# ingonyama-zk/gnark-icicle

Measured on AMD Instinct MI355X. Metric: BN254 G1 MSM Mpoints/s (2^20 points per GPU, sharded MSM), higher is better.
Workload: dtype u32 limbs (BN254 Fp/Fr Montgomery, integer); 1 GPU; BN254 G1 MSM 2^20 random points/scalars per GPU (BASELINE configs[1]); points_per_gpu=1048576, total_points=1048576, parallelism=msm-shard1

## Files before the change

### gnark-icicle_amd/csrc/msm.hpp

```cpp
#pragma once
#include <algorithm>
#include <cmath>
#include <cstddef>
#include <cstdint>
#include <cstdlib>
#include <hip/hip_runtime.h>
#include "curves.hpp"

struct gm_ctx;
struct gm_msm_pending;

namespace gm {
struct Arena;
constexpr uint32_t S2_BIG = 1u << 16;
constexpr uint32_t S2_STAGE = 6144;
struct SortGeom {
  uint32_t T = 0, F = 0, G = 0, NC = 0, NS = 0;
  size_t M = 0;
  bool compact = false;
};
inline bool sort_compact_fits(uint32_t F, uint32_t G, size_t npts) {
  uint32_t vb = 1;
  while (npts && ((npts - 1) >> (vb - 1))) vb++;
  return F + G + vb <= 32;
}
int msm_sort_digits(gm_ctx* ctx, Arena& arena, const SortGeom& g, size_t n, uint32_t W, uint32_t nb,
                    uint32_t shared_stride, const uint32_t* dig, const uint32_t* scount, uint32_t* keys_out,
                    uint32_t* vals_out, uint32_t* offsets);

constexpr uint32_t PRECOMP_LAYOUT = 2;
struct MsmPrecomp {
  uint32_t c = 0, W = 0;
  uint32_t narrow = 0;
  size_t stride = 0;
};
inline uint32_t precomp_narrow(uint32_t c, uint32_t W, int bits) {
  const long long e = (long long)c * W - (bits + 1);
  if (e <= 0) return 0;
  return (uint32_t)(e < (long long)W - 1 ? e : (long long)W - 1);
}

MsmPrecomp msm_choose_precomp(size_t n, int bits);

inline int choose_window(size_t n, int bits) {
  int best = 8;
  double best_cost = 1e300;
  for (int c = 8; c <= 20; c++) {
    const double W = (double)((bits + 1 + c - 1) / c);
    const double cost = (double)n * W + 3.0 * W * (double)(1u << (c - 1));
    if (cost < best_cost) {
      best_cost = cost;
      best = c;
    }
  }
  return best;
}

constexpr int GLV_HALF_BITS = 127;

struct MsmPlanGeom {
  size_t n = 0;
  int bits = 0;
  uint32_t c = 0, W = 0, nb = 0, Wred = 0, total = 0;
  uint32_t wn = 0;
  size_t npts = 0, M = 0;
  SortGeom sg;
};
inline const char* msm_plan_geom(size_t n0, int fr_bits, bool glv, const MsmPrecomp* pre, int c_override,
                                 MsmPlanGeom& g) {
  g = MsmPlanGeom();
  size_t n = n0;
  g.bits = fr_bits;
  if (glv) {
    n = 2 * n0;
    g.bits = GLV_HALF_BITS;
  }
  g.n = n;
  if (n >= (size_t(1) << 31)) return "msm: n must be < 2^31";
  const bool shared = pre && pre->c;
  if (shared && (pre->stride < n || (size_t)pre->W * pre->stride >= (size_t(1) << 31) || pre->narrow >= pre->W ||
                 (size_t)pre->c * pre->W - pre->narrow < (size_t)fr_bits + 1))
    return "msm: precomputed point set does not cover this MSM";
  const uint32_t c = shared ? pre->c : (c_override ? (uint32_t)c_override : (uint32_t)choose_window(n, g.bits));
  const uint32_t W = shared ? pre->W : (uint32_t)(g.bits + 1 + c - 1) / c;
  g.c = c;
  g.W = W;
  g.nb = 1u << (c - 1);
  g.Wred = shared ? 1 : W;
  g.total = g.Wred * g.nb;
  g.npts = shared ? (size_t)W * pre->stride : n;
  const size_t M = (size_t)W * n;
  g.M = M;
  if (M >= (size_t(1) << 31)) return "msm: n * windows must be < 2^31";
  SortGeom& sg = g.sg;
  sg.T = g.total;
  sg.M = M;
  sg.F = 4;
  const double bin_entries = glv || shared ? 4096.0 : 2048.0;
  while (sg.F < 13 && (double)M * std::ldexp(1.0, (int)sg.F + 1) <= bin_entries * sg.T) sg.F++;
  auto bins = [&](uint32_t sh) { return (uint32_t)(((uint64_t)sg.T + (1ull << sh) - 1) >> sh); };
  auto touched = [&](uint32_t sh) { return shared ? bins(sh) : std::max(1u, g.nb >> sh); };
  const char* ming = getenv("GM_MSM_SORT_MING");
  sg.G = ming ? (uint32_t)std::min(10, std::max(0, atoi(ming))) : 0u;
  const uint32_t max_touched = (shared && M < (size_t(1) << 24)) ? 8192u : 512u;
  while (sg.G < 10 && (touched(sg.F + sg.G) > max_touched || bins(sg.F + sg.G) > 8192)) sg.G++;
  while (sg.G && sg.F + sg.G > 31) sg.G--;
  sg.NC = bins(sg.F);
  sg.NS = bins(sg.F + sg.G);
  if (sg.NS > 8192) return "msm: too many buckets for the sort";
  const char* wide = getenv("GM_MSM_SORT_WIDE");
  sg.compact = !(wide && atoi(wide) > 0) && sort_compact_fits(sg.F, sg.G, g.npts);
  g.wn = shared ? W - pre->narrow : W;
  if (!shared && !glv) {
    const uint32_t narrow = c * W - (uint32_t)(g.bits + 1);
    if (narrow < W) g.wn = W - narrow;
  }
  return nullptr;
}

inline void msm_seg_geom(uint32_t Wred, uint32_t nb, uint32_t& L, uint32_t& nseg) {
  uint32_t Lwant = 4;
  while (Lwant < 32 && (size_t)Wred * nb / (2 * Lwant) >= (size_t(1) << 17)) Lwant *= 2;
  L = nb >= Lwant ? Lwant : nb;
  nseg = nb / L;
}

constexpr uint32_t BS_THREADS = 256;
struct MsmTreeGeom {
  static constexpr uint32_t MAX_LEVELS = 24;
  uint32_t levels = 0, lg[MAX_LEVELS] = {}, Q = 2;
};
inline bool msm_tree_geom(uint32_t nseg, size_t xyzz_bytes, MsmTreeGeom& g) {
  g = MsmTreeGeom();
  const size_t slot_budget = (96u << 10) / xyzz_bytes;
  uint32_t m = nseg, Q = 2;
  while (m > 1) {
    uint32_t lg = 0;
    while ((2u << lg) <= m && (size_t)(2u << lg) * Q <= slot_budget && (1u << lg) * (Q + 1) <= 2 * BS_THREADS) lg++;
    if (lg == 0 || g.levels == MsmTreeGeom::MAX_LEVELS) return false;
    g.lg[g.levels++] = lg;
    Q += lg;
    m >>= lg;
  }
  g.Q = Q;
  return true;
}

constexpr uint32_t MSM_SKIP = 0x7fffffffu;

struct MsmPlan {
  uint32_t c = 0, W = 0, nb = 0, total = 0;
  uint32_t Wred = 0;
  size_t n = 0, M = 0;
  size_t npts = 0;
  int bits = 0;
  uint32_t wn = 0;
  uint32_t* keys = nullptr;
  uint32_t* vals = nullptr;
  uint32_t* offsets = nullptr;
  uint32_t T = 0;
  size_t max_pieces = 0, max_parts = 0;
  uint4* pieces = nullptr;
  uint32_t* pcount = nullptr;
  uint32_t* pbase = nullptr;
  uint32_t* partb = nullptr;
};
constexpr uint32_t PIECE_PART = 0x80000000u;
constexpr uint32_t PIECE_MAX_LEN = 128;
uint32_t msm_piece_len(const gm_ctx* ctx, size_t M);
int msm_piece_plan(gm_ctx* ctx, Arena& arena, MsmPlan& plan, uint32_t T);
template <class C>
int msm_plan(gm_ctx* ctx, Arena& arena, const void* scalars_dev, size_t n, const MsmPrecomp* pre,
             MsmPlan& plan, bool glv = false, bool pieces = true, bool keys = true);
bool msm_glv_on(const gm_ctx* ctx, bool g2, size_t n);
template <class C, bool G2>
int msm_run(gm_ctx* ctx, const MsmPlan& plan, const void* points_internal,
            typename GroupSel<C, G2>::HF (&jac_out)[3]);

struct MsmTail {
  size_t n = 0, M = 0;
  uint32_t c = 0, W = 0, Wr = 0, nb = 0, total = 0, L = 0, nseg = 0, K = 0, Q = 2;
  uint32_t wn = 0;
  const uint32_t* keys = nullptr;
  const uint32_t* offsets = nullptr;
  uint32_t T = 0;
  size_t max_parts = 0;
  const uint32_t *pcount = nullptr, *pbase = nullptr, *partb = nullptr;
  void *buckets = nullptr, *pfirst = nullptr, *plast = nullptr, *nodes_a = nullptr, *nodes_b = nullptr;
  void *wsum = nullptr, *errw = nullptr;
  uint8_t* stage = nullptr;
  gm_ctx* stage_ctx = nullptr;
  int stage_idx = -1;
  hipEvent_t done = nullptr;
  void release_stage();
  MsmTail() = default;
  MsmTail(const MsmTail&) = delete;
  MsmTail& operator=(const MsmTail&) = delete;
  ~MsmTail() {
    if (done) hipEventDestroy(done);
    release_stage();
  }
};
template <class C, bool G2>
int msm_launch(gm_ctx* ctx, Arena& arena, const MsmPlan& plan, const void* points_internal, MsmTail& t);
template <class C, bool G2>
int msm_finish(gm_ctx* ctx, MsmTail& t, typename GroupSel<C, G2>::HF (&jac_out)[3]);
template <class C, bool G2>
int msm_device_launch(gm_ctx* ctx, Arena& arena, const void* scalars_dev, const void* points_dev, size_t n,
                      bool points_internal, const MsmPrecomp* pre, MsmTail& t,
                      hipEvent_t inputs_read = nullptr);

template <class C, bool G2>
int msm_device(gm_ctx* ctx, const void* scalars_dev, const void* points_dev, size_t n,
               typename GroupSel<C, G2>::HF (&jac_out)[3], bool points_internal = false,
               const MsmPrecomp* pre = nullptr);
template <class C, bool G2>
int msm_prepare_points(gm_ctx* ctx, const void* gnark_points, size_t n, void* dst);
template <class C, bool G2>
int msm_precompute_points(gm_ctx* ctx, const void* gnark_points, size_t n, const MsmPrecomp& pre, void* dst);
template <class C, bool G2>
size_t msm_internal_point_bytes();
int msm_async_queue(gm_ctx* ctx, int curve, int g2, const void* scalars_dev, const void* points_dev, size_t n,
                    bool prepared, gm_msm_pending** out);
}
```

### gnark-icicle_amd/csrc/msm_impl.hpp

```cpp
#pragma once
#include "curves.hpp"
#include "msm.hpp"
#include "pair_fp2.hpp"
#include "runtime.hpp"

#include <hip/hip_ext.h>

#include <cmath>
#include <cstdlib>
#include <cstring>
#include <type_traits>

namespace gm {

template <class Fr>
GM_DEV uint32_t window_bits(const FeG<Fr>& k, uint32_t bit, uint32_t mask) {
  const uint32_t idx = bit >> 5, sh = bit & 31;
  uint32_t lo = 0, hi = 0;
#pragma unroll
  for (int i = 0; i < Fr::NG; i++) {
    lo = (idx == (uint32_t)i) ? k.w[i] : lo;
    hi = (idx + 1 == (uint32_t)i) ? k.w[i] : hi;
  }
  const uint64_t v = ((uint64_t)hi << 32) | lo;
  return (uint32_t)(v >> sh) & mask;
}

template <class Fr>
GM_DEV FeG<Fr> load_scalar_canonical(const uint32_t* __restrict__ s, uint32_t i) {
  return fe_pack(fe_gnark_to_canonical(fe_load_g<Fr>(s, i)));
}

struct DigitGeom {
  uint32_t n, c, W, nb, shared_stride, F;
  uint32_t wn;
};
GM_HD void window_geom(uint32_t c, uint32_t wn, uint32_t w, uint32_t& off, uint32_t& cw) {
  off = w * c - (w > wn ? w - wn : 0u);
  cw = w >= wn ? c - 1 : c;
}

constexpr uint32_t DG_THREADS = 1024, DG_PPT = 4;

template <class Fr>
__global__ void __launch_bounds__(1024) k_msm_digits(const uint32_t* __restrict__ scalars, DigitGeom g,
                                                     uint32_t NC, uint32_t* __restrict__ dig,
                                                     uint32_t* __restrict__ ccount) {
  extern __shared__ uint32_t dg_lds[];
  const uint32_t t = threadIdx.x;
  for (uint32_t q = t; q < NC; q += DG_THREADS) dg_lds[q] = 0;
  __syncthreads();
  const uint32_t base = blockIdx.x * DG_THREADS * DG_PPT;
  for (uint32_t r = 0; r < DG_PPT; r++) {
    const uint32_t i = base + r * DG_THREADS + t;
    if (i >= g.n) break;
    const FeG<Fr> k = load_scalar_canonical<Fr>(scalars, i);
    uint32_t carry = 0;
    for (uint32_t w = 0; w < g.W; w++) {
      uint32_t off, cw;
      window_geom(g.c, g.wn, w, off, cw);
      const uint32_t raw = window_bits(k, off, (1u << cw) - 1) + carry;
      uint32_t d, neg;
      if (raw > (1u << (cw - 1))) {
        d = (1u << cw) - raw;
        carry = 1;
        neg = 1;
      } else {
        d = raw;
        carry = 0;
        neg = 0;
      }
      dig[(size_t)w * g.n + i] = d ? (d - 1) | (neg << 31) : 0xffffffffu;
      if (d) atomicAdd(&dg_lds[(g.shared_stride ? d - 1 : w * g.nb + d - 1) >> g.F], 1u);
    }
  }
  __syncthreads();
  for (uint32_t q = t; q < NC; q += DG_THREADS)
    if (dg_lds[q]) atomicAdd(&ccount[q], dg_lds[q]);
}

struct GlvBn254 {
  GM_HD static constexpr uint64_t g1(int i) {
    constexpr uint64_t a[5] = {0x163b4843cb4b9a5eull, 0x149d540fd5e495ccull, 0x5398fd0300ff6565ull,
                               0x4ccef014a773d2d2ull, 0x0000000000000002ull};
    return a[i];
  }
  GM_HD static constexpr uint64_t g2(int i) {
    constexpr uint64_t a[4] = {0x8fa7d32d2fafba64ull, 0x6eb9c714773a6ef2ull, 0xd91d232ec7e0b3d7ull,
                               0x0000000000000002ull};
    return a[i];
  }
  static constexpr uint64_t A1_LO = 0x8211bbeb7d4f1128ull, A1_HI = 0x6f4d8248eeb859fcull;
  static constexpr uint64_t A2 = 0x89d3256894d213e3ull;
  static constexpr uint64_t B2_LO = 0x0be4e1541221250bull, B2_HI = 0x6f4d8248eeb859fdull;
  GM_HD static constexpr uint32_t beta29(int i) {
    constexpr uint32_t a[9] = {0x18ccb791u, 0x175b1c3au, 0x0b83d6e2u, 0x0e8ed071u, 0x1282bee2u,
                               0x04220e84u, 0x1fe4017fu, 0x15084d4au, 0x00169119u};
    return a[i];
  }
  GM_HD static constexpr uint32_t beta29_g2(int i) {
    constexpr uint32_t a[9] = {0x0a337995u, 0x158d1d23u, 0x189c9b98u, 0x12fa4e45u, 0x185faadcu,
                               0x0176f16du, 0x0eed93bau, 0x14291140u, 0x000c0afeu};
    return a[i];
  }
};

struct GlvBls377 {
  GM_HD static constexpr uint64_t g(int i) {
    constexpr uint64_t a[5] = {0x5cc5a03b7b820d29ull, 0x3366fc876f25c6b5ull, 0x7f72ed32af90182cull,
                               0xb3f7aa969fd37160ull, 0x0000000000000003ull};
    return a[i];
  }
  static constexpr uint64_t LAM_LO = 0x0a11800000000000ull, LAM_HI = 0x452217cc90000001ull;
  GM_HD static constexpr uint32_t beta29(int i) {
    constexpr uint32_t a[14] = {0x1c8a7893u, 0x0b7d08f2u, 0x06b88506u, 0x162aa2edu, 0x1c5fdf80u,
                                0x11b95a22u, 0x03b86dd7u, 0x1191f770u, 0x10701220u, 0x1501c11fu,
                                0x1cee88bbu, 0x118d05ecu, 0x06f2fa26u, 0x00000000u};
    return a[i];
  }
  GM_HD static constexpr uint32_t beta29_g2(int i) {
    constexpr uint32_t a[14] = {0x098a903fu, 0x0deef70eu, 0x0bd62e43u, 0x12fc3bfau, 0x0de940feu,
                                0x047b8e82u, 0x17ec1b27u, 0x1a776815u, 0x120a67b5u, 0x0a70d0c4u,
                                0x0271dc9au, 0x182f7308u, 0x19602487u, 0x00000000u};
    return a[i];
  }
};

struct GlvBls381 {
  GM_HD static constexpr uint64_t g(int i) {
    constexpr uint64_t a[5] = {0xda5e4f8d896c72ddull, 0x389f49a7268bf7a3ull, 0x63f6e522f6cfee30ull,
                               0x7c6becf1e01faaddull, 0x0000000000000001ull};
    return a[i];
  }
  static constexpr uint64_t LAM_LO = 0x00000000ffffffffull, LAM_HI = 0xac45a4010001a402ull;
  GM_HD static constexpr uint64_t r(int i) {
    constexpr uint64_t a[4] = GM_BLS12381_FR_P64;
    return a[i];
  }
  GM_HD static constexpr uint64_t half(int i) {
    constexpr uint64_t a[4] = {0x7fffffff80000000ull, 0xa9ded2017fff2dffull, 0x199cec0404d0ec02ull,
                               0x39f6d3a994cebea4ull};
    return a[i];
  }
  static constexpr unsigned __int128 MAX_HALF =
      ((((unsigned __int128)LAM_HI << 64) | LAM_LO) + 1) / 2 + 1;
  static_assert(MAX_HALF < ((unsigned __int128)1 << GLV_HALF_BITS),
                "the halves of the balanced split must fit the digits of a GLV plan");
  GM_HD static constexpr uint32_t beta29(int i) {
    constexpr uint32_t a[14] = {0x1195dfebu, 0x1b04e484u, 0x06026044u, 0x086070a2u, 0x1fd68858u,
                                0x137e9670u, 0x06871e67u, 0x1e736664u, 0x083b24f6u, 0x08a70373u,
                                0x02a012fdu, 0x0112f94bu, 0x18a2733cu, 0x00000003u};
    return a[i];
  }
  GM_HD static constexpr uint32_t beta29_g2(int i) {
    constexpr uint32_t a[14] = {0x0abf79e7u, 0x194b14ebu, 0x1ceb16a6u, 0x1845cd5du, 0x0c814568u,
                                0x199ca109u, 0x13ee6ee1u, 0x05d123e5u, 0x0dfbdce2u, 0x010ecb54u,
                                0x0d9337edu, 0x1daaf4b0u, 0x146806fbu, 0x0000000cu};
    return a[i];
  }
};

template <class P>
struct GlvBeta;
template <>
struct GlvBeta<Bn254Fp> {
  GM_HD static constexpr uint32_t g1(int i) { return GlvBn254::beta29(i); }
  GM_HD static constexpr uint32_t g2(int i) { return GlvBn254::beta29_g2(i); }
};
template <>
struct GlvBeta<Bls377Fp> {
  GM_HD static constexpr uint32_t g1(int i) { return GlvBls377::beta29(i); }
  GM_HD static constexpr uint32_t g2(int i) { return GlvBls377::beta29_g2(i); }
};
template <>
struct GlvBeta<Bls381Fp> {
  GM_HD static constexpr uint32_t g1(int i) { return GlvBls381::beta29(i); }
  GM_HD static constexpr uint32_t g2(int i) { return GlvBls381::beta29_g2(i); }
};

template <class P>
GM_DEV Fe<P> glv_phi_x(const Fe<P>& x) {
  Fe<P> b;
#pragma unroll
  for (int j = 0; j < P::N; j++) b.v[j] = GlvBeta<P>::g1(j);
  return fe_mul(x, b);
}
template <class P, int B>
GM_DEV Fe2<P, B> glv_phi_x(const Fe2<P, B>& x) {
  Fe<P> b;
#pragma unroll
  for (int j = 0; j < P::N; j++) b.v[j] = GlvBeta<P>::g2(j);
  return {fe_mul(x.a0, b), fe_mul(x.a1, b)};
}

template <int NG, class GF>
GM_DEV unsigned __int128 glv_mulshift(const uint64_t (&k)[4], GF g) {
  uint64_t t[4 + NG] = {};
#pragma unroll
  for (int i = 0; i < 4; i++) {
    uint64_t carry = 0;
#pragma unroll
    for (int j = 0; j < NG; j++) {
      const unsigned __int128 v = (unsigned __int128)k[i] * g(j) + t[i + j] + carry;
      t[i + j] = (uint64_t)v;
      carry = (uint64_t)(v >> 64);
    }
    t[i + NG] = carry;
  }
  return ((unsigned __int128)t[7] << 64) | t[6];
}

template <class Fr>
GM_DEV void emit_digits(const FeG<Fr>& k, uint32_t flip, uint32_t i, const DigitGeom& g, uint32_t* __restrict__ dig,
                        uint32_t* lds) {
  const uint32_t mask = (1u << g.c) - 1;
  uint32_t carry = 0;
  for (uint32_t w = 0; w < g.W; w++) {
    const uint32_t raw = window_bits(k, w * g.c, mask) + carry;
    uint32_t d, neg;
    if (raw > g.nb) {
      d = (1u << g.c) - raw;
      carry = 1;
      neg = 1;
    } else {
      d = raw;
      carry = 0;
      neg = 0;
    }
    dig[(size_t)w * g.n + i] = d ? (d - 1) | ((neg ^ flip) << 31) : 0xffffffffu;
    if (d) atomicAdd(&lds[(w * g.nb + d - 1) >> g.F], 1u);
  }
}

template <class C>
struct Glv {
  static constexpr bool ok = false;
  static constexpr bool signed_k1 = false;
};
template <>
struct Glv<CurveBN254> {
  static constexpr bool ok = true;
  static constexpr bool signed_k1 = false;
  using U = unsigned __int128;
  GM_DEV static void split(const uint64_t (&k64)[4], U& k1, U& k2, uint32_t& neg2) {
    const U c1 = glv_mulshift<5>(k64, GlvBn254::g1);
    const U c2 = glv_mulshift<4>(k64, GlvBn254::g2);
    const U a1 = ((U)GlvBn254::A1_HI << 64) | GlvBn254::A1_LO;
    const U b2 = ((U)GlvBn254::B2_HI << 64) | GlvBn254::B2_LO;
    const U klo = ((U)k64[1] << 64) | k64[0];
    k1 = klo - c1 * a1 - c2 * (U)GlvBn254::A2;
    k2 = c1 * (U)GlvBn254::A2 - c2 * b2;
    neg2 = (uint32_t)(k2 >> 127);
    if (neg2) k2 = (U)0 - k2;
  }
};
template <>
struct Glv<CurveBLS12377> {
  static constexpr bool ok = true;
  static constexpr bool signed_k1 = false;
  using U = unsigned __int128;
  GM_DEV static void split(const uint64_t (&k64)[4], U& k1, U& k2, uint32_t& neg2) {
    U q = glv_mulshift<5>(k64, GlvBls377::g);
    const U lam = ((U)GlvBls377::LAM_HI << 64) | GlvBls377::LAM_LO;
    const U klo = ((U)k64[1] << 64) | k64[0];
    U r = klo - q * lam;
    if (r >= lam) {
      r -= lam;
      q += 1;
    }
    k1 = r;
    k2 = q;
    neg2 = 0;
  }
};

template <>
struct Glv<CurveBLS12381> {
  static constexpr bool ok = true;
  static constexpr bool signed_k1 = true;
  using U = unsigned __int128;
  GM_DEV static void split(const uint64_t (&k64)[4], U& k1, uint32_t& neg1, U& k2, uint32_t& neg2) {
    uint64_t kk[4], borrow = 0, b2 = 0;
#pragma unroll
    for (int i = 0; i < 4; i++) {
      const U d = (U)GlvBls381::half(i) - k64[i] - borrow;
      borrow = (uint64_t)(d >> 127) & 1;
      const U e = (U)GlvBls381::r(i) - k64[i] - b2;
      b2 = (uint64_t)(e >> 127) & 1;
      kk[i] = (uint64_t)e;
    }
    const uint32_t flip = (uint32_t)borrow;
#pragma unroll
    for (int i = 0; i < 4; i++) kk[i] = flip ? kk[i] : k64[i];
    U q = glv_mulshift<5>(kk, GlvBls381::g);
    const U lam = ((U)GlvBls381::LAM_HI << 64) | GlvBls381::LAM_LO;
    const U klo = ((U)kk[1] << 64) | kk[0];
    U r0 = klo - q * lam;
    neg1 = 0;
    if (r0 > (lam >> 1)) {
      r0 = lam - r0;
      q += 1;
      neg1 = 1;
    }
    k1 = r0;
    k2 = q;
    neg1 ^= flip;
    neg2 = flip;
  }
};

template <class C>
__global__ void __launch_bounds__(1024) k_msm_digits_glv(const uint32_t* __restrict__ scalars, DigitGeom g,
                                                         uint32_t n0, uint32_t NC, uint32_t* __restrict__ dig,
                                                         uint32_t* __restrict__ ccount) {
  using Fr = typename C::Fr;
  extern __shared__ uint32_t dg_lds[];
  const uint32_t t = threadIdx.x;
  for (uint32_t q = t; q < NC; q += DG_THREADS) dg_lds[q] = 0;
  __syncthreads();
  const uint32_t base = blockIdx.x * DG_THREADS * DG_PPT;
  for (uint32_t r = 0; r < DG_PPT; r++) {
    const uint32_t i = base + r * DG_THREADS + t;
    if (i >= n0) break;
    const FeG<Fr> k = load_scalar_canonical<Fr>(scalars, i);
    uint64_t k64[4];
#pragma unroll
    for (int j = 0; j < 4; j++) k64[j] = (uint64_t)k.w[2 * j] | ((uint64_t)k.w[2 * j + 1] << 32);
    unsigned __int128 k1, k2;
    uint32_t neg1 = 0, neg2;
    if constexpr (Glv<C>::signed_k1) Glv<C>::split(k64, k1, neg1, k2, neg2);
    else Glv<C>::split(k64, k1, k2, neg2);
    FeG<Fr> m1, m2;
#pragma unroll
    for (int j = 0; j < Fr::NG; j++) {
      m1.w[j] = j < 4 ? (uint32_t)(k1 >> (32 * j)) : 0u;
      m2.w[j] = j < 4 ? (uint32_t)(k2 >> (32 * j)) : 0u;
    }
    emit_digits<Fr>(m1, neg1, i, g, dig, dg_lds);
    emit_digits<Fr>(m2, neg2, n0 + i, g, dig, dg_lds);
  }
  __syncthreads();
  for (uint32_t q = t; q < NC; q += DG_THREADS)
    if (dg_lds[q]) atomicAdd(&ccount[q], dg_lds[q]);
}

template <class F, bool GLV>
__global__ void __launch_bounds__(256) k_msm_convert_points_lds(const uint32_t* __restrict__ src, size_t n,
                                                                uint32_t* __restrict__ dst) {
  constexpr int PW = 2 * Coord<F>::WORDS;
  constexpr uint32_t Q = PW / 4;
  static_assert(PW % 4 == 0, "points are whole uint4s");
  __shared__ uint4 tile[256 * (Q + 1)];
  const size_t b0 = (size_t)blockIdx.x * 256;
  const uint32_t np = (uint32_t)min((size_t)256, n - b0);
  const uint32_t t = threadIdx.x;
  const uint4* s = reinterpret_cast<const uint4*>(src) + b0 * Q;
  for (uint32_t q = t; q < np * Q; q += 256) tile[(q / Q) * (Q + 1) + q % Q] = s[q];
  __syncthreads();
  uint32_t* mine = reinterpret_cast<uint32_t*>(tile + t * (Q + 1));
  Affine<F> a;
  if (t < np) {
    a = load_affine_gnark<F>(mine);
    store_affine_packed<F>(mine, a);
  }
  __syncthreads();
  uint4* d = reinterpret_cast<uint4*>(dst) + b0 * Q;
  for (uint32_t q = t; q < np * Q; q += 256) d[q] = tile[(q / Q) * (Q + 1) + q % Q];
  if constexpr (GLV) {
    __syncthreads();
    if (t < np) {
      a.x = glv_phi_x(a.x);
      store_affine_packed<F>(mine, a);
    }
    __syncthreads();
    uint4* d2 = reinterpret_cast<uint4*>(dst) + (n + b0) * Q;
    for (uint32_t q = t; q < np * Q; q += 256) d2[q] = tile[(q / Q) * (Q + 1) + q % Q];
  }
}

template <class F>
__global__ void __launch_bounds__(256) k_msm_convert_points(const uint32_t* __restrict__ src, size_t n,
                                                            uint32_t* __restrict__ dst) {
  const size_t i = (size_t)blockIdx.x * blockDim.x + threadIdx.x;
  if (i >= n) return;
  constexpr int PW = 2 * Coord<F>::WORDS;
  store_affine_packed<F>(dst + i * PW, load_affine_gnark<F>(src + i * PW));
}

template <class F>
__global__ void __launch_bounds__(128) k_msm_precompute(uint32_t* __restrict__ pts, size_t n, size_t stride,
                                                        uint32_t c, uint32_t W, uint32_t wn) {
  const size_t i = (size_t)blockIdx.x * blockDim.x + threadIdx.x;
  if (i >= n) return;
  constexpr int PW = 2 * Coord<F>::WORDS;
  const Affine<F> P = load_affine_packed<F>(pts + i * PW);
  Affine<F> zero;
  zero.x = FOps<F>::zero();
  zero.y = FOps<F>::zero();
  if (aff_is_inf(P)) {
    for (uint32_t w = 1; w < W; w++) store_affine_packed<F>(pts + (w * stride + i) * PW, zero);
    return;
  }
  XYZZ<F> acc;
  acc.x = P.x;
  acc.y = P.y;
  acc.zz = FOps<F>::one();
  acc.zzz = FOps<F>::one();
  for (uint32_t w = 1; w < W; w++) {
    const uint32_t cw = (w - 1 >= wn) ? c - 1 : c;
    for (uint32_t k = 0; k < cw; k++) acc = xyzz_dbl(acc);
    Affine<F> r = zero;
    if (!xyzz_is_inf(acc)) {
      const F t = fe_inv(fe_mul(acc.zz, acc.zzz));
      r.x = fe_mul(acc.x, fe_mul(t, acc.zzz));
      r.y = fe_mul(acc.y, fe_mul(t, acc.zz));
    }
    store_affine_packed<F>(pts + (w * stride + i) * PW, r);
  }
}

template <int PW>
struct PackedPt {
  uint32_t w[PW];
};
template <int PW>
GM_DEV PackedPt<PW> load_packed_pt(const uint32_t* __restrict__ src) {
  static_assert(PW % 4 == 0, "packed points are whole 16-byte chunks");
  PackedPt<PW> r;
#pragma unroll
  for (int q = 0; q < PW / 4; q++) {
    const uint4 v = reinterpret_cast<const uint4*>(src)[q];
    r.w[4 * q] = v.x;
    r.w[4 * q + 1] = v.y;
    r.w[4 * q + 2] = v.z;
    r.w[4 * q + 3] = v.w;
  }
  return r;
}

template <class F>
struct LazyAcc {
  static constexpr bool on = false;
  template <bool CH = false>
  GM_DEV static void add(XYZZ<F>& a, Affine<F> p, bool neg) {
    if (neg) p.y = fe_neg(p.y);
    xyzz_add_aff(a, p);
  }
};
template <class P>
struct LazyAcc<Fe<P>> {
  static constexpr bool on = true;
  template <bool CH = false>
  GM_DEV static void add(XYZZ<Fe<P>>& a, const Affine<Fe<P>>& p, bool neg) {
    xyzz_add_aff_lz<P, CH ? 2 : 0>(a, p, neg);
  }
};

GM_DEV void wave_stamp_begin(unsigned long long* stamp) {
  if (stamp && blockIdx.x < 64 && (threadIdx.x & 63) == 0)
    atomicMin(stamp + blockIdx.x * 32, (unsigned long long)wall_clock64());
}
GM_DEV void wave_stamp_end(unsigned long long* stamp) {
  if (stamp && (threadIdx.x & 63) == 0)
    atomicMax(stamp + (blockIdx.x & 63) * 32 + 1, (unsigned long long)wall_clock64());
}

struct __attribute__((packed, aligned(4))) EntryQuad {
  uint32_t x, y, z, w;
};
GM_DEV uint4 load_entry_quad(const uint32_t* __restrict__ p) {
  const EntryQuad q = *reinterpret_cast<const EntryQuad*>(p);
  return make_uint4(q.x, q.y, q.z, q.w);
}

template <int PW, bool PREFETCH>
GM_DEV bool accum_next(const uint32_t* __restrict__ points, uint32_t n, const uint32_t* __restrict__ vp,
                       uint32_t len, uint32_t q, uint4& vg, uint32_t& vn, PackedPt<PW>& Pn,
                       uint32_t* __restrict__ err) {
  if ((q & 3) == 3) {
    if (q + 1 < len) vg = load_entry_quad(vp + q + 1);
  } else {
    vg = make_uint4(vg.y, vg.z, vg.w, vg.w);
  }
  vn = vg.x;
  if (q + 1 < len) {
    if ((vn & 0x7fffffffu) >= n) {
      atomicOr(err, 2u);
      return false;
    }
    if (PREFETCH) Pn = load_packed_pt<PW>(points + (size_t)(vn & 0x7fffffffu) * PW);
  }
  return true;
}

template <class F, bool CH, bool PREFETCH = false>
GM_DEV void accum_piece_body(const uint32_t* __restrict__ points, uint32_t n, const uint32_t* __restrict__ vals,
                             const uint4* __restrict__ pieces, const uint32_t* __restrict__ pcount,
                             XYZZ<F>* __restrict__ buckets, XYZZ<F>* __restrict__ parts,
                             uint32_t* __restrict__ err) {
  const uint32_t t = blockIdx.x * blockDim.x + threadIdx.x;
  if (t >= pcount[0]) return;
  const uint32_t* vp = vals + pieces[t].x;
  const uint32_t len = pieces[t].y;
  uint4 vg = load_entry_quad(vp);
  uint32_t v = vg.x;
  if ((v & 0x7fffffffu) >= n) {
    atomicOr(err, 2u);
    return;
  }
  constexpr int PW = 2 * Coord<F>::WORDS;
  PackedPt<PW> P, Pn;
  if (PREFETCH) P = load_packed_pt<PW>(points + (size_t)(v & 0x7fffffffu) * PW);
  XYZZ<F> acc = xyzz_inf<F>();
  for (uint32_t q = 0; q < len; q++) {
    uint32_t vn;
    if (!accum_next<PW, PREFETCH>(points, n, vp, len, q, vg, vn, Pn, err)) return;
    if (!PREFETCH) P = load_packed_pt<PW>(points + (size_t)(v & 0x7fffffffu) * PW);
    LazyAcc<F>::template add<CH>(acc, load_affine_packed<F>(P.w), (v >> 31) != 0);
    v = vn;
    if (PREFETCH) P = Pn;
  }
  const uint32_t dst = pieces[t].z;
  *((dst & PIECE_PART) ? parts + (dst & ~PIECE_PART) : buckets + dst) = acc;
}

template <class F>
__global__ void __launch_bounds__(128) __attribute__((amdgpu_waves_per_eu(4)))
k_msm_accum_seg_ch(const uint32_t* __restrict__ points, uint32_t n, const uint32_t* __restrict__ vals,
                   const uint4* __restrict__ pieces, const uint32_t* __restrict__ pcount,
                   XYZZ<F>* __restrict__ buckets, XYZZ<F>* __restrict__ parts, uint32_t* __restrict__ err,
                   unsigned long long* __restrict__ stamp) {
  wave_stamp_begin(stamp);
  accum_piece_body<F, true>(points, n, vals, pieces, pcount, buckets, parts, err);
  wave_stamp_end(stamp);
}
template <class F>
struct AccumW4 {
  static constexpr bool ok = false;
};
template <class P>
struct AccumW4<Fe<P>> {
  static constexpr bool ok = P::N <= 9;
};
template <class F>
__global__ void __launch_bounds__(128) k_msm_accum_seg_pf4(const uint32_t* __restrict__ points, uint32_t n,
                                                           const uint32_t* __restrict__ vals,
                                                           const uint4* __restrict__ pieces,
                                                           const uint32_t* __restrict__ pcount,
                                                           XYZZ<F>* __restrict__ buckets,
                                                           XYZZ<F>* __restrict__ parts,
                                                           uint32_t* __restrict__ err,
                                                           unsigned long long* __restrict__ stamp) {
  wave_stamp_begin(stamp);
  accum_piece_body<F, false, true>(points, n, vals, pieces, pcount, buckets, parts, err);
  wave_stamp_end(stamp);
}
template <class F>
constexpr auto g1_accum_kernel() {
  if constexpr (AccumW4<F>::ok) return k_msm_accum_seg_ch<F>;
  else return k_msm_accum_seg_pf4<F>;
}

template <class F>
struct PairSel {
  static constexpr bool ok = false;
};
template <class P, int B>
struct PairSel<Fe2<P, B>> {
  static constexpr bool ok = true;
  static constexpr auto kernel() {
    if constexpr (P::N <= 9) return k_msm_accum_seg_pair<P, B, false, 3, true, true>;
    else return k_msm_accum_seg_pair<P, B, false, GM_PAIR_WPE, true>;
  }
  static constexpr auto fixup() { return k_msm_fixup_pair<P, B>; }
  static constexpr auto fixup_edge() { return k_msm_fixup_edge_pair<P, B>; }
  static constexpr auto fix_tree() { return k_msm_fix_tree_pair<P, B>; }
  static constexpr auto fixup_long() { return k_msm_fixup_long_pair<P, B>; }
  static constexpr auto seg() { return k_msm_seg_pair<P, B>; }
  static constexpr auto bitsum() { return k_msm_bitsum_pair<P, B>; }
};
template <class F>
constexpr bool kOneLane = !PairSel<F>::ok;

template <class F>
struct FullAdd {
  GM_DEV static XYZZ<F> add(const XYZZ<F>& a, const XYZZ<F>& b) { return xyzz_add(a, b); }
  GM_DEV static XYZZ<F> canon(const XYZZ<F>& a) { return a; }
  GM_DEV static XYZZ<F> canon2(const XYZZ<F>& a) { return a; }
};
template <class P>
struct FullAdd<Fe<P>> {
  GM_DEV static XYZZ<Fe<P>> add(const XYZZ<Fe<P>>& a, const XYZZ<Fe<P>>& b) { return xyzz_add_lz(a, b); }
  GM_DEV static XYZZ<Fe<P>> canon(const XYZZ<Fe<P>>& a) { return xyzz_canon_raw(a); }
  GM_DEV static XYZZ<Fe<P>> canon2(const XYZZ<Fe<P>>& a) { return xyzz_canon2(a); }
};

constexpr uint32_t FIX_SERIAL = 8;

template <class F>
__global__ void __launch_bounds__(128) k_msm_fixup(const uint32_t* __restrict__ offsets, uint32_t total,
                                                   uint32_t T, XYZZ<F>* __restrict__ buckets,
                                                   const XYZZ<F>* __restrict__ parts,
                                                   const uint32_t* __restrict__ pbase,
                                                   uint32_t* __restrict__ maxspan) {
  const uint32_t b = blockIdx.x * blockDim.x + threadIdx.x;
  if (b >= total) return;
  const uint32_t len = offsets[b + 1] - offsets[b];
  if (len <= T) return;
  const uint32_t p = (len + T - 1) / T;
  if (p - 1 > FIX_SERIAL) {
    atomicMax(maxspan, p - 1);
    return;
  }
  const XYZZ<F>* q = parts + pbase[b];
  XYZZ<F> acc = q[0];
  for (uint32_t i = 1; i < p; i++) acc = FullAdd<F>::add(acc, q[i]);
  buckets[b] = acc;
}

template <class F>
__global__ void __launch_bounds__(128) k_msm_fix_tree(const uint32_t* __restrict__ offsets, uint32_t T,
                                                      const uint32_t* __restrict__ pcount,
                                                      const uint32_t* __restrict__ pbase,
                                                      const uint32_t* __restrict__ partb, uint32_t d,
                                                      XYZZ<F>* __restrict__ parts) {
  const uint32_t s = blockIdx.x * blockDim.x + threadIdx.x;
  if (s >= pcount[1]) return;
  const uint32_t b = partb[s];
  const uint32_t p = (offsets[b + 1] - offsets[b] + T - 1) / T;
  if (p - 1 <= FIX_SERIAL) return;
  const uint32_t rel = s - pbase[b], step = 1u << d;
  if ((rel & ((step << 1) - 1)) == 0 && rel + step < p) parts[s] = FullAdd<F>::add(parts[s], parts[s + step]);
}

template <class F>
__global__ void __launch_bounds__(128) k_msm_fixup_long(const uint32_t* __restrict__ offsets, uint32_t total,
                                                        uint32_t T, XYZZ<F>* __restrict__ buckets,
                                                        const XYZZ<F>* __restrict__ parts,
                                                        const uint32_t* __restrict__ pbase) {
  const uint32_t b = blockIdx.x * blockDim.x + threadIdx.x;
  if (b >= total) return;
  const uint32_t len = offsets[b + 1] - offsets[b];
  if (len <= T || (len + T - 1) / T - 1 <= FIX_SERIAL) return;
  buckets[b] = parts[pbase[b]];
}

template <class F>
__global__ void __launch_bounds__(128) k_msm_seg(const XYZZ<F>* __restrict__ buckets,
                                                 const uint32_t* __restrict__ offsets, uint32_t nb, uint32_t L,
                                                 uint32_t nseg, uint32_t W, XYZZ<F>* __restrict__ nodes) {
  const uint32_t t = blockIdx.x * blockDim.x + threadIdx.x;
  if (t >= W * nseg) return;
  const uint32_t w = t / nseg, s = t % nseg;
  const size_t b0 = (size_t)w * nb + (size_t)s * L;
  const XYZZ<F>* B = buckets + b0;
  const uint32_t* O = offsets + b0;
  uint32_t o_hi = O[L];
  uint32_t o_lo = O[L - 1];
  XYZZ<F> S = o_lo == o_hi ? xyzz_inf<F>() : B[L - 1], T = S;
  for (int j = (int)L - 2; j >= 0; j--) {
    o_hi = o_lo;
    o_lo = O[j];
    S = FullAdd<F>::add(S, o_lo == o_hi ? xyzz_inf<F>() : B[j]);
    T = FullAdd<F>::add(T, S);
  }
  nodes[2 * (size_t)t] = FullAdd<F>::canon(S);
  nodes[2 * (size_t)t + 1] = FullAdd<F>::canon(T);
}

template <class F>
__global__ void __launch_bounds__(BS_THREADS) k_msm_bitsum(const XYZZ<F>* __restrict__ in, uint32_t m,
                                                    uint32_t Qin, uint32_t NT, uint32_t lgNT,
                                                    XYZZ<F>* __restrict__ out) {
  extern __shared__ __attribute__((aligned(16))) char smem_raw[];
  XYZZ<F>* X = reinterpret_cast<XYZZ<F>*>(smem_raw);
  const uint32_t groups = m / NT;
  const uint32_t w = blockIdx.x / groups, j = blockIdx.x % groups;
  const XYZZ<F>* src = in + ((size_t)w * m + (size_t)j * NT) * Qin;
  for (uint32_t q = threadIdx.x; q < NT * Qin; q += blockDim.x) X[q] = src[q];
  __syncthreads();
  for (uint32_t d = 0; d < lgNT; d++) {
    const uint32_t qc = Qin + d + 1;
    const uint32_t tasks = (NT >> (d + 1)) * qc;
    const uint32_t child = (Qin << d);
    XYZZ<F> r0, r1;
    uint32_t s0 = 0xffffffffu, s1 = 0xffffffffu;
    {
      const uint32_t t = threadIdx.x;
      if (t < tasks) {
        const uint32_t p = t / qc, q = t % qc, base = p * 2 * child;
        r0 = (q + 1 < qc) ? FullAdd<F>::canon2(FullAdd<F>::add(X[base + q], X[base + child + q])) : X[base + child];
        s0 = base + q;
      }
    }
    {
      const uint32_t t = threadIdx.x + blockDim.x;
      if (t < tasks) {
        const uint32_t p = t / qc, q = t % qc, base = p * 2 * child;
        r1 = (q + 1 < qc) ? FullAdd<F>::canon2(FullAdd<F>::add(X[base + q], X[base + child + q])) : X[base + child];
        s1 = base + q;
      }
    }
    __syncthreads();
    if (s0 != 0xffffffffu) X[s0] = r0;
    if (s1 != 0xffffffffu) X[s1] = r1;
    __syncthreads();
  }
  const uint32_t Qout = Qin + lgNT;
  XYZZ<F>* dst = out + ((size_t)w * groups + j) * Qout;
  for (uint32_t q = threadIdx.x; q < Qout; q += blockDim.x) dst[q] = X[q];
}

template <class F>
__global__ void __launch_bounds__(128) k_msm_export(const XYZZ<F>* __restrict__ nodes, uint32_t count,
                                                    uint32_t* __restrict__ out) {
  const uint32_t t = blockIdx.x * blockDim.x + threadIdx.x;
  if (t >= count) return;
  uint32_t* o = out + (size_t)t * 4 * Coord<F>::WORDS;
  const XYZZ<F> r = nodes[t];
  Coord<F>::store_gnark(o, r.x);
  Coord<F>::store_gnark(o + Coord<F>::WORDS, r.y);
  Coord<F>::store_gnark(o + 2 * Coord<F>::WORDS, r.zz);
  Coord<F>::store_gnark(o + 3 * Coord<F>::WORDS, r.zzz);
}

template <class C>
int msm_plan(gm_ctx* ctx, Arena& arena, const void* scalars_dev, size_t n, const MsmPrecomp* pre,
             MsmPlan& plan, bool glv, bool pieces, bool keys) {
  hipStream_t st = ctx->stream;
  plan = MsmPlan();
  plan.n = n;
  plan.bits = C::FR_BITS;
  if (n == 0) return GM_OK;
  if (glv && (!Glv<C>::ok || (pre && pre->c))) {
    set_error("msm: the GLV split needs a plain (not precomputed) layout");
    return GM_ERR_INVALID;
  }
  const size_t n0 = n;
  MsmPlanGeom pg;
  const char* refusal = msm_plan_geom(n0, C::FR_BITS, glv, pre, ctx->msm_c_override, pg);
  n = pg.n;
  plan.n = pg.n;
  plan.bits = pg.bits;
  plan.c = pg.c;
  plan.W = pg.W;
  plan.nb = pg.nb;
  plan.Wred = pg.Wred;
  plan.total = pg.total;
  plan.npts = pg.npts;
  plan.M = pg.M;
  if (refusal) {
    set_error(refusal);
    return GM_ERR_INVALID;
  }
  const bool shared = pre && pre->c;
  const uint32_t c = pg.c, W = pg.W;
  const size_t M = pg.M;
  const SortGeom& sg = pg.sg;
  int rc;
  DevBuf dig, keys_out, vals_out, offsets, scount;
  if ((rc = dig.alloc(arena, sizeof(uint32_t) * M)) || (keys && (rc = keys_out.alloc(arena, sizeof(uint32_t) * M))) ||
      (rc = vals_out.alloc(arena, sizeof(uint32_t) * M + 16)) ||
      (rc = offsets.alloc(arena, sizeof(uint32_t) * ((size_t)plan.total + 1))) ||
      (rc = scount.alloc(arena, sizeof(uint32_t) * sg.NS)))
    return rc;
  DigitGeom g;
  g.n = (uint32_t)n;
  g.c = c;
  g.W = W;
  g.nb = plan.nb;
  g.shared_stride = shared ? (uint32_t)pre->stride : 0u;
  g.wn = pg.wn;
  plan.wn = g.wn;
  g.F = sg.F + sg.G;
  {
    ProfScope ps(ctx, "msm_digits");
    GM_HIP(hipMemsetAsync(scount.p, 0, sizeof(uint32_t) * sg.NS, st));
    if constexpr (Glv<C>::ok) {
      if (glv)
        hipLaunchKernelGGL(k_msm_digits_glv<C>, dim3(blocks_for(n0, DG_THREADS * DG_PPT)), dim3(DG_THREADS),
                         sizeof(uint32_t) * sg.NS, st, reinterpret_cast<const uint32_t*>(scalars_dev), g,
                           (uint32_t)n0, sg.NS, dig.as<uint32_t>(), scount.as<uint32_t>());
    }
    if (!glv)
      hipLaunchKernelGGL(k_msm_digits<typename C::Fr>, dim3(blocks_for(n, DG_THREADS * DG_PPT)), dim3(DG_THREADS),
                         sizeof(uint32_t) * sg.NS, st, reinterpret_cast<const uint32_t*>(scalars_dev), g, sg.NS,
                         dig.as<uint32_t>(), scount.as<uint32_t>());
    GM_HIP(hipGetLastError());
  }
  {
    ProfScope ps(ctx, "msm_sort");
    if (ctx->profiling) ctx->stats[sg.compact ? "msm_sort_compact" : "msm_sort_wide"].count += 1;
    if ((rc = msm_sort_digits(ctx, arena, sg, n, W, plan.nb, g.shared_stride, dig.as<uint32_t>(),
                              scount.as<uint32_t>(), keys_out.as<uint32_t>(), vals_out.as<uint32_t>(),
                              offsets.as<uint32_t>())))
      return rc;
  }
  plan.keys = keys_out.as<uint32_t>();
  plan.vals = vals_out.as<uint32_t>();
  plan.offsets = offsets.as<uint32_t>();
  if (pieces) {
    ProfScope ps(ctx, "msm_piece_plan");
    if ((rc = msm_piece_plan(ctx, arena, plan, msm_piece_len(ctx, M)))) return rc;
  }
  return GM_OK;
}

template <class C, bool G2>
int msm_reduce(gm_ctx* ctx, MsmTail& t) {
  using DF = typename GroupSel<C, G2>::DF;
  hipStream_t st = ctx->stream;
  ProfScope ps(ctx, "msm_bucket_reduce");
  uint32_t Q = 2;
  constexpr bool pairs = PairSel<DF>::ok;
  if constexpr (PairSel<DF>::ok) {
    if (pairs)
      hipLaunchKernelGGL(PairSel<DF>::seg(), dim3(blocks_for(2 * (size_t)t.Wr * t.nseg, 128)), dim3(128), 0, st,
                         (const uint32_t*)t.buckets, (const uint32_t*)t.offsets, t.nb, t.L, t.nseg, t.Wr,
                         (uint32_t*)t.nodes_a);
  }
  if constexpr (kOneLane<DF>) {
    if (!pairs)
      hipLaunchKernelGGL(k_msm_seg<DF>, dim3(blocks_for((size_t)t.Wr * t.nseg, 128)), dim3(128), 0, st,
                         (const XYZZ<DF>*)t.buckets, (const uint32_t*)t.offsets, t.nb, t.L, t.nseg, t.Wr,
                         (XYZZ<DF>*)t.nodes_a);
  }
  MsmTreeGeom tg;
  if (!msm_tree_geom(t.nseg, sizeof(XYZZ<DF>), tg)) {
    set_error("msm: bucket reduction does not fit LDS");
    return GM_ERR_INVALID;
  }
  uint32_t m = t.nseg;
  XYZZ<DF>* cur = (XYZZ<DF>*)t.nodes_a;
  XYZZ<DF>* nxt = (XYZZ<DF>*)t.nodes_b;
  for (uint32_t lv = 0; lv < tg.levels; lv++) {
    const uint32_t lg = tg.lg[lv];
    const uint32_t NT = 1u << lg;
    const uint32_t groups = m / NT;
    if constexpr (PairSel<DF>::ok) {
      if (pairs)
        hipLaunchKernelGGL(PairSel<DF>::bitsum(), dim3(t.Wr * groups), dim3(BS_PAIR_THREADS), sizeof(XYZZ<DF>) * NT * Q,
                           st, (const uint32_t*)cur, m, Q, NT, lg, (uint32_t*)nxt);
    }
    if constexpr (kOneLane<DF>) {
      if (!pairs)
        hipLaunchKernelGGL(k_msm_bitsum<DF>, dim3(t.Wr * groups), dim3(BS_THREADS), sizeof(XYZZ<DF>) * NT * Q, st,
                           cur, m, Q, NT, lg, nxt);
    }
    Q += lg;
    m = groups;
    std::swap(cur, nxt);
  }
  hipLaunchKernelGGL(k_msm_export<DF>, dim3(blocks_for((size_t)t.Wr * Q, 128)), dim3(128), 0, st, cur, t.Wr * Q,
                     (uint32_t*)t.wsum);
  GM_HIP(hipGetLastError());
  t.Q = Q;
  return GM_OK;
}

template <class C, bool G2>
int msm_fix_long(gm_ctx* ctx, MsmTail& t, uint32_t maxspan) {
  using DF = typename GroupSel<C, G2>::DF;
  hipStream_t st = ctx->stream;
  if constexpr (PairSel<DF>::ok) {
    {
      const size_t nslices = (t.M + t.K - 1) / t.K;
      for (uint32_t d = 0; (1u << d) < maxspan; d++)
        hipLaunchKernelGGL(PairSel<DF>::fix_tree(), dim3(blocks_for(2 * nslices, 128)), dim3(128), 0, st, t.keys,
                           t.offsets, t.total, t.K, (uint32_t)nslices, d, (uint32_t*)t.pfirst, FIX_SERIAL);
      hipLaunchKernelGGL(PairSel<DF>::fixup_long(), dim3(blocks_for(2 * (size_t)t.total, 128)), dim3(128), 0, st,
                         t.offsets, t.total, t.K, (uint32_t*)t.buckets, (const uint32_t*)t.pfirst,
                         (const uint32_t*)t.plast, FIX_SERIAL);
      GM_HIP(hipGetLastError());
      return GM_OK;
    }
  }
  if constexpr (kOneLane<DF>) {
    for (uint32_t d = 0; (1u << d) <= maxspan; d++)
      hipLaunchKernelGGL(k_msm_fix_tree<DF>, dim3(blocks_for(t.max_parts, 128)), dim3(128), 0, st, t.offsets, t.T,
                         t.pcount, t.pbase, t.partb, d, (XYZZ<DF>*)t.pfirst);
    hipLaunchKernelGGL(k_msm_fixup_long<DF>, dim3(blocks_for(t.total, 128)), dim3(128), 0, st, t.offsets, t.total,
                       t.T, (XYZZ<DF>*)t.buckets, (const XYZZ<DF>*)t.pfirst, t.pbase);
  }
  GM_HIP(hipGetLastError());
  return GM_OK;
}

template <class C, bool G2>
int msm_readback(gm_ctx* ctx, MsmTail& t) {
  using DF = typename GroupSel<C, G2>::DF;
  constexpr int WORDS = Coord<DF>::WORDS;
  hipStream_t st = ctx->stream;
  const size_t wbytes = sizeof(uint32_t) * 4 * WORDS * t.Wr * t.Q;
  if (!t.stage) {
    if (int r = tail_pinned_acquire(ctx, 16 + wbytes, &t.stage, &t.stage_idx)) return r;
    t.stage_ctx = ctx;
  }
  GM_HIP(hipMemcpyAsync(t.stage, t.errw, 16, hipMemcpyDeviceToHost, st));
  GM_HIP(hipMemcpyAsync(t.stage + 16, t.wsum, wbytes, hipMemcpyDeviceToHost, st));
  if (!t.done) GM_HIP(hipEventCreateWithFlags(&t.done, hipEventDisableTiming));
  GM_HIP(hipEventRecord(t.done, st));
  return GM_OK;
}

template <class C, bool G2>
int msm_launch(gm_ctx* ctx, Arena& arena, const MsmPlan& plan, const void* points_internal, MsmTail& t) {
  using DF = typename GroupSel<C, G2>::DF;
  using HF = typename GroupSel<C, G2>::HF;
  hipStream_t st = ctx->stream;
  t.n = plan.n;
  if (plan.n == 0) return GM_OK;
  t.c = plan.c;
  t.W = plan.W;
  t.wn = plan.wn;
  t.nb = plan.nb;
  t.total = plan.total;
  t.Wr = plan.Wred;
  t.M = plan.M;
  t.keys = plan.keys;
  t.offsets = plan.offsets;
  msm_seg_geom(t.Wr, t.nb, t.L, t.nseg);
  t.K = 64u;
  if (!G2) {
    if (!plan.T || !plan.pieces) {
      set_error("msm: the plan has no piece plan (built for G2 only)");
      return GM_ERR_INVALID;
    }
    t.T = plan.T;
    t.max_parts = plan.max_parts;
    t.pcount = plan.pcount;
    t.pbase = plan.pbase;
    t.partb = plan.partb;
  } else if (!plan.keys) {
    set_error("msm: the plan has no sorted keys (built for G1 only)");
    return GM_ERR_INVALID;
  }
  int rc;
  constexpr int WORDS = Coord<DF>::WORDS;
  static_assert(sizeof(HF) == 4 * WORDS, "host/device layout mismatch");
  const size_t nslices = G2 ? (t.M + t.K - 1) / t.K : plan.max_parts;
  DevBuf buckets, nodes_a, nodes_b, wsum, errw, pfirst, plast;
  if ((rc = errw.alloc(arena, 16)) || (rc = buckets.alloc(arena, sizeof(XYZZ<DF>) * (size_t)t.total)) ||
      (rc = nodes_a.alloc(arena, sizeof(XYZZ<DF>) * 2 * (size_t)t.Wr * t.nseg)) ||
      (rc = nodes_b.alloc(arena, sizeof(XYZZ<DF>) * 2 * (size_t)t.Wr * t.nseg)) ||
      (rc = wsum.alloc(arena, sizeof(uint32_t) * 4 * WORDS * t.Wr * (2 + t.c))) ||
      (rc = pfirst.alloc(arena, sizeof(XYZZ<DF>) * nslices)) ||
      (rc = plast.alloc(arena, G2 ? sizeof(XYZZ<DF>) * nslices : 16)))
    return rc;
  t.buckets = buckets.p;
  t.nodes_a = nodes_a.p;
  t.nodes_b = nodes_b.p;
  t.wsum = wsum.p;
  t.errw = errw.p;
  t.pfirst = pfirst.p;
  t.plast = plast.p;
  GM_HIP(hipMemsetAsync(errw.p, 0, 16, st));
  {
    if (ctx->acc_chain) {
      if (!ctx->acc_tail) GM_HIP(hipEventCreateWithFlags(&ctx->acc_tail, hipEventDisableTiming));
      else GM_HIP(hipStreamWaitEvent(st, ctx->acc_tail, 0));
    }
    struct TailMark {
      gm_ctx* c;
      hipStream_t s;
      ~TailMark() {
        if (c->acc_chain) hipEventRecord(c->acc_tail, s);
      }
    } tail_mark{ctx, st};
    ProfScope ps(ctx, G2 ? "msm_accum_g2" : "msm_accum_g1", true);
    if constexpr (PairSel<DF>::ok) {
      hipExtLaunchKernelGGL(PairSel<DF>::kernel(), dim3(blocks_for(2 * nslices, 128)), dim3(128), 0, st, ps.a, ps.b,
                            0, reinterpret_cast<const uint32_t*>(points_internal), (uint32_t)plan.npts, plan.keys,
                            plan.vals, plan.offsets, t.total, t.K, buckets.as<uint32_t>(), pfirst.as<uint32_t>(),
                            plast.as<uint32_t>(), errw.as<uint32_t>());
    } else {
      hipExtLaunchKernelGGL(g1_accum_kernel<DF>(), dim3(blocks_for(plan.max_pieces, 128)), dim3(128), 0, st, ps.a,
                            ps.b, 0, reinterpret_cast<const uint32_t*>(points_internal), (uint32_t)plan.npts,
                            plan.vals, plan.pieces, plan.pcount, buckets.as<XYZZ<DF>>(), pfirst.as<XYZZ<DF>>(),
                            errw.as<uint32_t>(), ps.wave_stamp("msm_accum_g1_exec"));
    }
  }
  {
    ProfScope ps(ctx, "msm_fixup");
    if constexpr (PairSel<DF>::ok) {
      if (plan.M < (size_t)t.K * t.total) {
        if (nslices > 1)
          hipLaunchKernelGGL(PairSel<DF>::fixup_edge(), dim3(blocks_for(2 * (nslices - 1), 128)), dim3(128), 0, st,
                             plan.keys, plan.offsets, t.total, t.K, (uint32_t)nslices, buckets.as<uint32_t>(),
                             pfirst.as<uint32_t>(), plast.as<uint32_t>(), errw.as<uint32_t>() + 1, FIX_SERIAL);
      } else {
        hipLaunchKernelGGL(PairSel<DF>::fixup(), dim3(blocks_for(2 * (size_t)t.total, 128)), dim3(128), 0, st,
                           plan.offsets, t.total, t.K, buckets.as<uint32_t>(), pfirst.as<uint32_t>(),
                           plast.as<uint32_t>(), errw.as<uint32_t>() + 1, FIX_SERIAL);
      }
    } else if (plan.M > t.T) {
      hipLaunchKernelGGL(k_msm_fixup<DF>, dim3(blocks_for(t.total, 128)), dim3(128), 0, st, plan.offsets, t.total,
                         t.T, buckets.as<XYZZ<DF>>(), pfirst.as<XYZZ<DF>>(), plan.pbase, errw.as<uint32_t>() + 1);
    }
  }
  {
    double fullest = 0;
    for (uint32_t w = 0; w < t.W; w++) {
      uint32_t off, cw;
      window_geom(t.c, plan.wn, w, off, cw);
      const int left = plan.bits - (int)off;
      const double h = std::ldexp(1.0, std::max(0, std::min((int)cw - 1, left)));
      const double load = (double)plan.n / h;
      fullest = t.Wr == 1 ? fullest + load : std::max(fullest, load);
    }
    if (fullest > 0.5 * FIX_SERIAL * (G2 ? t.K : t.T)) {
      uint8_t* pb;
      int pbi;
      if ((rc = tail_pinned_acquire(ctx, 16, &pb, &pbi))) return rc;
      const hipError_t e1 = hipMemcpyAsync(pb, errw.p, 16, hipMemcpyDeviceToHost, st);
      const hipError_t e2 = e1 == hipSuccess ? hipStreamSynchronize(st) : e1;
      uint32_t ms;
      memcpy(&ms, pb + 4, 4);
      tail_pinned_release(ctx, pbi);
      GM_HIP(e2);
      if (ms > FIX_SERIAL) {
        if ((rc = msm_fix_long<C, G2>(ctx, t, ms))) return rc;
        GM_HIP(hipMemsetAsync(errw.as<uint32_t>() + 1, 0, 4, st));
      }
    }
  }
  if ((rc = msm_reduce<C, G2>(ctx, t))) return rc;
  return msm_readback<C, G2>(ctx, t);
}

template <class C, bool G2>
int msm_finish(gm_ctx* ctx, MsmTail& t, typename GroupSel<C, G2>::HF (&jac_out)[3]) {
  using HF = typename GroupSel<C, G2>::HF;
  using HJ = host::Jac<HF>;
  if (t.n == 0) {
    HJ inf = HJ::inf();
    jac_out[0] = inf.x;
    jac_out[1] = inf.y;
    jac_out[2] = inf.z;
    return GM_OK;
  }
  int rc;
  GM_HIP(hipEventSynchronize(t.done));
  uint32_t herr, maxspan;
  memcpy(&herr, t.stage, 4);
  memcpy(&maxspan, t.stage + 4, 4);
  if (maxspan > FIX_SERIAL) {
    if ((rc = msm_fix_long<C, G2>(ctx, t, maxspan)) || (rc = msm_reduce<C, G2>(ctx, t)) ||
        (rc = msm_readback<C, G2>(ctx, t)))
      return rc;
    GM_HIP(hipEventSynchronize(t.done));
    memcpy(&herr, t.stage, 4);
  }
  if (herr) {
    set_error("msm: internal consistency check failed (code " + std::to_string(herr) + ")");
    return GM_ERR_DEVICE;
  }
  const uint32_t Wr = t.Wr, Q = t.Q, c = t.c;
  std::vector<HF> hw(4 * (size_t)Wr * Q);
  memcpy(hw.data(), t.stage + 16, sizeof(HF) * hw.size());
  t.release_stage();
  uint32_t lgL = 0;
  while ((1u << lgL) < t.L) lgL++;
  const int top = (int)(c * Wr);
  std::vector<std::vector<uint32_t>> at(top + 1);
  for (uint32_t w = 0; w < Wr; w++) {
    uint32_t off, cw;
    window_geom(c, Wr == 1 ? 1u : t.wn, w, off, cw);
    at[off].push_back(w * Q + 1);
    for (uint32_t b = 0; b + 2 < Q; b++) at[off + lgL + b].push_back(w * Q + 2 + b);
  }
  HJ acc = HJ::inf();
  for (int e = top; e >= 0; e--) {
    if (!acc.is_inf()) acc = host::jdbl(acc);
    for (uint32_t id : at[e]) {
      const HF* p = &hw[4 * (size_t)id];
      if (p[2].is_zero()) continue;
      acc = host::jadd(acc, host::xyzz_to_jac(p[0], p[1], p[2], p[3]));
    }
  }
  jac_out[0] = acc.x;
  jac_out[1] = acc.y;
  jac_out[2] = acc.z;
  return GM_OK;
}

template <class C, bool G2>
int msm_run(gm_ctx* ctx, const MsmPlan& plan, const void* points_internal,
            typename GroupSel<C, G2>::HF (&jac_out)[3]) {
  Arena arena(ctx);
  MsmTail t;
  int rc = msm_launch<C, G2>(ctx, arena, plan, points_internal, t);
  return rc ? rc : msm_finish<C, G2>(ctx, t, jac_out);
}

template <class C, bool G2>
int msm_device_launch(gm_ctx* ctx, Arena& arena, const void* scalars_dev, const void* points_dev, size_t n,
                      bool points_internal, const MsmPrecomp* pre, MsmTail& t, hipEvent_t inputs_read) {
  using DF = typename GroupSel<C, G2>::DF;
  int rc;
  const void* pts = points_dev;
  DevBuf ipts;
  bool glv = false;
  if (!points_internal && n) {
    if (pre && pre->c) {
      set_error("msm: a precomputed point set must be device-internal");
      return GM_ERR_INVALID;
    }
    glv = Glv<C>::ok && msm_glv_on(ctx, G2, n);
    if ((rc = ipts.alloc(arena, 2 * Coord<DF>::WORDS * sizeof(uint32_t) * n * (glv ? 2 : 1)))) return rc;
    ProfScope ps(ctx, "msm_convert_points");
    const uint32_t* src = reinterpret_cast<const uint32_t*>(points_dev);
    if (glv)
      hipLaunchKernelGGL((k_msm_convert_points_lds<DF, true>), dim3(blocks_for(n, 256)), dim3(256), 0, ctx->stream,
                         src, n, ipts.as<uint32_t>());
    else
      hipLaunchKernelGGL((k_msm_convert_points_lds<DF, false>), dim3(blocks_for(n, 256)), dim3(256), 0, ctx->stream,
                         src, n, ipts.as<uint32_t>());
    pts = ipts.p;
  }
  MsmPlan plan;
  if ((rc = msm_plan<C>(ctx, arena, scalars_dev, n, pre, plan, glv, !G2, G2))) return rc;
  if (inputs_read) GM_HIP(hipEventRecord(inputs_read, ctx->stream));
  return msm_launch<C, G2>(ctx, arena, plan, pts, t);
}

template <class C, bool G2>
int msm_device(gm_ctx* ctx, const void* scalars_dev, const void* points_dev, size_t n,
               typename GroupSel<C, G2>::HF (&jac_out)[3], bool points_internal, const MsmPrecomp* pre) {
  Arena arena(ctx);
  MsmTail t;
  int rc = msm_device_launch<C, G2>(ctx, arena, scalars_dev, points_dev, n, points_internal, pre, t);
  return rc ? rc : msm_finish<C, G2>(ctx, t, jac_out);
}

template <class C, bool G2>
size_t msm_internal_point_bytes() {
  return 2 * Coord<typename GroupSel<C, G2>::DF>::WORDS * sizeof(uint32_t);
}

template <class C, bool G2>
int msm_prepare_points(gm_ctx* ctx, const void* gnark_points, size_t n, void* dst) {
  using DF = typename GroupSel<C, G2>::DF;
  if (n == 0) return GM_OK;
  hipLaunchKernelGGL(k_msm_convert_points<DF>, dim3(blocks_for(n, 256)), dim3(256), 0, ctx->stream,
                     reinterpret_cast<const uint32_t*>(gnark_points), n, reinterpret_cast<uint32_t*>(dst));
  GM_HIP(hipGetLastError());
  return GM_OK;
}

template <class C, bool G2>
int msm_precompute_points(gm_ctx* ctx, const void* gnark_points, size_t n, const MsmPrecomp& pre, void* dst) {
  using DF = typename GroupSel<C, G2>::DF;
  if (n == 0) return GM_OK;
  if (pre.stride < n || pre.W == 0 || pre.c == 0) {
    set_error("msm precompute: bad layout");
    return GM_ERR_INVALID;
  }
  hipLaunchKernelGGL(k_msm_convert_points<DF>, dim3(blocks_for(n, 256)), dim3(256), 0, ctx->stream,
                     reinterpret_cast<const uint32_t*>(gnark_points), n, reinterpret_cast<uint32_t*>(dst));
  if (pre.W > 1)
    hipLaunchKernelGGL(k_msm_precompute<DF>, dim3(blocks_for(n, 128)), dim3(128), 0, ctx->stream,
                       reinterpret_cast<uint32_t*>(dst), n, pre.stride, pre.c, pre.W, pre.W - pre.narrow);
  GM_HIP(hipGetLastError());
  return GM_OK;
}

#define GM_MSM_INSTANTIATE(C, G2)                                                              \
  template size_t msm_internal_point_bytes<C, G2>();                                          \
  template int msm_prepare_points<C, G2>(gm_ctx*, const void*, size_t, void*);                \
  template int msm_precompute_points<C, G2>(gm_ctx*, const void*, size_t, const MsmPrecomp&, void*); \
  template int msm_run<C, G2>(gm_ctx*, const MsmPlan&, const void*, typename GroupSel<C, G2>::HF (&)[3]); \
  template int msm_launch<C, G2>(gm_ctx*, Arena&, const MsmPlan&, const void*, MsmTail&);      \
  template int msm_finish<C, G2>(gm_ctx*, MsmTail&, typename GroupSel<C, G2>::HF (&)[3]);     \
  template int msm_device_launch<C, G2>(gm_ctx*, Arena&, const void*, const void*, size_t, bool, \
                                        const MsmPrecomp*, MsmTail&, hipEvent_t);              \
  template int msm_device<C, G2>(gm_ctx*, const void*, const void*, size_t,                    \
                                 typename GroupSel<C, G2>::HF (&)[3], bool, const MsmPrecomp*);
#define GM_MSM_INSTANTIATE_PLAN(C) \
  template int msm_plan<C>(gm_ctx*, Arena&, const void*, size_t, const MsmPrecomp*, MsmPlan&, bool, bool, bool);

}
```

### gnark-icicle_amd/csrc/msm_sort.hip

```cpp
#include "msm.hpp"
#include "runtime.hpp"
#include "scan.hpp"
#include "sort_util.hpp"

namespace gm {

template <class E>
struct SortEnt;
template <>
struct SortEnt<uint64_t> {
  __device__ __forceinline__ static uint64_t make(uint32_t b, uint32_t v, uint32_t) { return ((uint64_t)v << 32) | b; }
  __device__ __forceinline__ static uint32_t low(uint64_t e) { return (uint32_t)e; }
  __device__ __forceinline__ static uint32_t val(uint64_t e, uint32_t) { return (uint32_t)(e >> 32); }
};
template <>
struct SortEnt<uint32_t> {
  __device__ __forceinline__ static uint32_t make(uint32_t b, uint32_t v, uint32_t kb) {
    return (b & ((1u << kb) - 1)) | ((v & 0x7fffffffu) << kb) | (v & 0x80000000u);
  }
  __device__ __forceinline__ static uint32_t low(uint32_t e) { return e; }
  __device__ __forceinline__ static uint32_t val(uint32_t e, uint32_t kb) {
    return ((e & 0x7fffffffu) >> kb) | (e & 0x80000000u);
  }
};

static size_t device_lds_per_block(int device) {
  static std::mutex mu;
  static std::map<int, size_t> cache;
  std::lock_guard<std::mutex> g(mu);
  auto it = cache.find(device);
  if (it != cache.end()) return it->second;
  int v = 0;
  if (hipDeviceGetAttribute(&v, hipDeviceAttributeMaxSharedMemoryPerBlock, device) != hipSuccess) {
    (void)hipGetLastError();
    v = 64 << 10;
  }
  return cache[device] = (size_t)v;
}

static __global__ void __launch_bounds__(1024) k_msm_s1_scan(const uint32_t* __restrict__ ccount, uint32_t NC,
                                                             uint32_t T, uint32_t psz, uint32_t* __restrict__ cbase,
                                                             uint32_t* __restrict__ ccursor,
                                                             uint32_t* __restrict__ pbase,
                                                             uint32_t* __restrict__ offsets) {
  __shared__ uint32_t a[8192];
  __shared__ uint32_t wsum[17];
  const uint32_t t = threadIdx.x;
  for (uint32_t q = t; q < NC; q += S_THREADS) a[q] = ccount[q];
  const uint32_t total = block_excl_scan(a, NC, wsum);
  for (uint32_t q = t; q < NC; q += S_THREADS) {
    cbase[q] = a[q];
    ccursor[q] = a[q];
    const uint32_t cnt = ccount[q];
    a[q] = cnt > psz ? (cnt + psz - 1) / psz : 1u;
  }
  if (t == 0) {
    cbase[NC] = total;
    offsets[T] = total;
  }
  const uint32_t parts = block_excl_scan(a, NC, wsum);
  for (uint32_t q = t; q < NC; q += S_THREADS) pbase[q] = a[q];
  if (t == 0) pbase[NC] = parts;
}

constexpr uint32_t S1_PPT = 8, S1_PTS = S_THREADS * S1_PPT;
template <class E>
static __global__ void __launch_bounds__(1024) k_msm_s1_scatter(const uint32_t* __restrict__ dig, uint32_t n,
                                                                uint32_t nb, uint32_t shared_stride, uint32_t F,
                                                                uint32_t NC, uint32_t nh,
                                                                uint32_t* __restrict__ ccursor,
                                                                E* __restrict__ tmp) {
  extern __shared__ uint32_t s1_lds[];
  uint32_t* hist = s1_lds;
  uint32_t* cur = s1_lds + nh;
  const uint32_t t = threadIdx.x, w = blockIdx.y, base = blockIdx.x * S1_PTS;
  const uint32_t wb = shared_stride ? 0u : w * nb;
  const uint32_t h0 = nh == NC ? 0u : wb >> F;
  for (uint32_t q = t; q < nh; q += S_THREADS) hist[q] = 0;
  __syncthreads();
  uint32_t dv[S1_PPT], rk[S1_PPT];
#pragma unroll
  for (uint32_t r = 0; r < S1_PPT; r++) {
    const uint32_t i = base + r * S_THREADS + t;
    dv[r] = i < n ? dig[(size_t)w * n + i] : 0xffffffffu;
    if (dv[r] != 0xffffffffu) rk[r] = lds_rank_add(hist, (((dv[r] & 0x7fffffffu) + wb) >> F) - h0);
  }
  __syncthreads();
  for (uint32_t q = t; q < nh; q += S_THREADS)
    if (hist[q]) cur[q] = atomicAdd(&ccursor[h0 + q], hist[q]);
  __syncthreads();
#pragma unroll
  for (uint32_t r = 0; r < S1_PPT; r++) {
    if (dv[r] == 0xffffffffu) continue;
    const uint32_t i = base + r * S_THREADS + t;
    const uint32_t b = (dv[r] & 0x7fffffffu) + wb;
    const uint32_t v = (shared_stride ? w * shared_stride + i : i) | (dv[r] & 0x80000000u);
    tmp[cur[(b >> F) - h0] + rk[r]] = SortEnt<E>::make(b, v, F);
  }
}

template <class E, uint32_t PPT>
static __global__ void __launch_bounds__(1024) k_msm_s1_scatter_st(const uint32_t* __restrict__ dig, uint32_t n,
                                                                   uint32_t nb, uint32_t shared_stride, uint32_t F,
                                                                   uint32_t NC, uint32_t nh,
                                                                   uint32_t* __restrict__ ccursor,
                                                                   E* __restrict__ tmp) {
  constexpr uint32_t PTS = S_THREADS * PPT;
  extern __shared__ uint64_t s1s_lds[];
  uint64_t* stage = s1s_lds;
  uint32_t* hist = reinterpret_cast<uint32_t*>(s1s_lds + PTS);
  uint32_t* cur = hist + nh;
  uint32_t* lb = cur + nh;
  uint32_t* wsum = lb + nh;
  const uint32_t t = threadIdx.x, w = blockIdx.y, base = blockIdx.x * PTS;
  const uint32_t wb = shared_stride ? 0u : w * nb;
  const uint32_t h0 = nh == NC ? 0u : wb >> F;
  for (uint32_t q = t; q < nh; q += S_THREADS) hist[q] = 0;
  __syncthreads();
  uint32_t dv[PPT], rk[PPT];
#pragma unroll
  for (uint32_t r = 0; r < PPT; r++) {
    const uint32_t i = base + r * S_THREADS + t;
    dv[r] = i < n ? dig[(size_t)w * n + i] : 0xffffffffu;
    if (dv[r] != 0xffffffffu) rk[r] = lds_rank_add(hist, (((dv[r] & 0x7fffffffu) + wb) >> F) - h0);
  }
  __syncthreads();
  for (uint32_t q = t; q < nh; q += S_THREADS) {
    const uint32_t h = hist[q];
    cur[q] = h ? atomicAdd(&ccursor[h0 + q], h) : 0u;
    lb[q] = h;
  }
  const uint32_t total = block_excl_scan(lb, nh, wsum);
#pragma unroll
  for (uint32_t r = 0; r < PPT; r++) {
    if (dv[r] == 0xffffffffu) continue;
    const uint32_t i = base + r * S_THREADS + t;
    const uint32_t b = (dv[r] & 0x7fffffffu) + wb;
    const uint32_t v = (shared_stride ? w * shared_stride + i : i) | (dv[r] & 0x80000000u);
    stage[lb[(b >> F) - h0] + rk[r]] = ((uint64_t)v << 32) | b;
  }
  __syncthreads();
  for (uint32_t q = t; q < total; q += S_THREADS) {
    const uint64_t e = stage[q];
    const uint32_t b = (uint32_t)e, h = (b >> F) - h0;
    tmp[cur[h] + (q - lb[h])] = SortEnt<E>::make(b, (uint32_t)(e >> 32), F);
  }
}

__device__ __forceinline__ void s2_locate(const uint32_t* __restrict__ pbase, uint32_t NC, uint32_t j, uint32_t* sh) {
  if (threadIdx.x == 0) {
    uint32_t lo = 0, hi = NC;
    if (pbase[NC] == NC) lo = j, hi = j + 1;
    while (hi - lo > 1) {
      const uint32_t mid = (lo + hi) >> 1;
      if (pbase[mid] <= j) lo = mid;
      else hi = mid;
    }
    sh[0] = lo;
    sh[1] = j - pbase[lo];
  }
  __syncthreads();
}

constexpr uint32_t SM_PART = 16384, SM_IPT = SM_PART / S_THREADS;

template <class E>
static __global__ void __launch_bounds__(1024) k_msm_sm_count(const E* __restrict__ tmp,
                                                              const uint32_t* __restrict__ sbase,
                                                              const uint32_t* __restrict__ spbase, uint32_t NS,
                                                              uint32_t F, uint32_t G, uint32_t* __restrict__ ccount) {
  __shared__ uint32_t hist[1024], sh[2];
  const uint32_t j = blockIdx.x, t = threadIdx.x;
  if (j >= spbase[NS]) return;
  s2_locate(spbase, NS, j, sh);
  const uint32_t s = sh[0], p = sh[1];
  const uint32_t start = sbase[s], cnt = sbase[s + 1] - start;
  const uint32_t lo = p * SM_PART, hi = min(lo + SM_PART, cnt), ng = 1u << G;
  for (uint32_t q = t; q < ng; q += S_THREADS) hist[q] = 0;
  __syncthreads();
  for (uint32_t e = lo + t; e < hi; e += S_THREADS) lds_rank_add(hist, (SortEnt<E>::low(tmp[start + e]) >> F) & (ng - 1));
  __syncthreads();
  for (uint32_t q = t; q < ng; q += S_THREADS)
    if (hist[q]) atomicAdd(&ccount[(s << G) + q], hist[q]);
}

static __global__ void __launch_bounds__(1024) k_msm_sm_scan(const uint32_t* __restrict__ ccount,
                                                             const uint32_t* __restrict__ sbase, uint32_t G,
                                                             uint32_t NC, uint32_t* __restrict__ cbase,
                                                             uint32_t* __restrict__ ccursor,
                                                             uint32_t* __restrict__ cparts) {
  __shared__ uint32_t a[1024], wsum[17];
  const uint32_t s = blockIdx.x, t = threadIdx.x, H0 = s << G;
  const uint32_t nh = min(1u << G, NC - H0);
  for (uint32_t q = t; q < nh; q += S_THREADS) a[q] = ccount[H0 + q];
  block_excl_scan(a, nh, wsum);
  for (uint32_t q = t; q < nh; q += S_THREADS) {
    const uint32_t c = ccount[H0 + q];
    cbase[H0 + q] = sbase[s] + a[q];
    ccursor[H0 + q] = sbase[s] + a[q];
    cparts[H0 + q] = c > S2_BIG ? (c + S2_BIG - 1) / S2_BIG : 1u;
  }
  if (t == 0 && H0 + nh == NC) cbase[NC] = sbase[s + 1];
}

template <class E>
static __global__ void __launch_bounds__(1024) k_msm_sm_scatter(const E* __restrict__ tmp,
                                                                const uint32_t* __restrict__ sbase,
                                                                const uint32_t* __restrict__ spbase, uint32_t NS,
                                                                uint32_t F, uint32_t G,
                                                                uint32_t* __restrict__ ccursor,
                                                                E* __restrict__ tmp2) {
  __shared__ uint32_t hist[1024], cur[1024], sh[2];
  const uint32_t j = blockIdx.x, t = threadIdx.x;
  if (j >= spbase[NS]) return;
  s2_locate(spbase, NS, j, sh);
  const uint32_t s = sh[0], p = sh[1];
  const uint32_t start = sbase[s], cnt = sbase[s + 1] - start;
  const uint32_t lo = p * SM_PART, hi = min(lo + SM_PART, cnt), ng = 1u << G;
  for (uint32_t q = t; q < ng; q += S_THREADS) hist[q] = 0;
  __syncthreads();
  E x[SM_IPT];
  uint32_t rk[SM_IPT];
#pragma unroll
  for (uint32_t it = 0; it < SM_IPT; it++) {
    const uint32_t e = lo + it * S_THREADS + t;
    if (e < hi) {
      x[it] = tmp[start + e];
      rk[it] = lds_rank_add(hist, (SortEnt<E>::low(x[it]) >> F) & (ng - 1));
    }
  }
  __syncthreads();
  for (uint32_t q = t; q < ng; q += S_THREADS)
    if (hist[q]) cur[q] = atomicAdd(&ccursor[(s << G) + q], hist[q]);
  __syncthreads();
#pragma unroll
  for (uint32_t it = 0; it < SM_IPT; it++) {
    const uint32_t e = lo + it * S_THREADS + t;
    if (e < hi) tmp2[cur[(SortEnt<E>::low(x[it]) >> F) & (ng - 1)] + rk[it]] = x[it];
  }
}

template <bool KEYS>
constexpr size_t s2_local_lds(uint32_t nf) {
  return sizeof(uint32_t) * (nf + (KEYS ? 2 : 1) * (size_t)S2_STAGE);
}
template <class E, bool KEYS>
static __global__ void __launch_bounds__(1024) k_msm_s2_local(const E* __restrict__ tmp,
                                                              const uint32_t* __restrict__ cbase,
                                                              const uint32_t* __restrict__ pbase, uint32_t NC,
                                                              uint32_t F, uint32_t kb, uint32_t T,
                                                              uint32_t* __restrict__ fcount,
                                                              uint32_t* __restrict__ keys_out,
                                                              uint32_t* __restrict__ vals_out,
                                                              uint32_t* __restrict__ offsets) {
  extern __shared__ uint32_t s2_lds[];
  __shared__ uint32_t sh[2], wsum[17];
  const uint32_t j = blockIdx.x, t = threadIdx.x;
  const uint32_t parts = pbase[NC];
  const uint32_t cj0 = j < NC ? cbase[j] : 0u, cj1 = j < NC ? cbase[j + 1] : 0u;
  if (j >= parts) return;
  uint32_t H, p, start, cnt;
  if (parts == NC) {
    H = j;
    p = 0;
    start = cj0;
    cnt = cj1 - cj0;
  } else {
    s2_locate(pbase, NC, j, sh);
    H = sh[0];
    p = sh[1];
    start = cbase[H];
    cnt = cbase[H + 1] - start;
  }
  const uint32_t b0 = H << F, nf = min(1u << F, T - b0), fmask = (1u << F) - 1;
  uint32_t* hist = s2_lds;
  for (uint32_t q = t; q < nf; q += S_THREADS) hist[q] = 0;
  __syncthreads();
  if (cnt <= S2_STAGE) {
    constexpr uint32_t IPT = S2_STAGE / S_THREADS;
    E x[IPT];
    uint32_t rk[IPT];
#pragma unroll
    for (uint32_t it = 0; it < IPT; it++) {
      const uint32_t e = it * S_THREADS + t;
      if (e < cnt) {
        x[it] = tmp[start + e];
        rk[it] = lds_rank_add(hist, SortEnt<E>::low(x[it]) & fmask);
      }
    }
    block_excl_scan(hist, nf, wsum);
    for (uint32_t f = t; f < nf; f += S_THREADS) offsets[b0 + f] = start + hist[f];
    uint32_t* sv = s2_lds + nf;
    uint32_t* sk = sv + S2_STAGE;
#pragma unroll
    for (uint32_t it = 0; it < IPT; it++) {
      const uint32_t e = it * S_THREADS + t;
      if (e < cnt) {
        const uint32_t f = SortEnt<E>::low(x[it]) & fmask;
        const uint32_t pos = hist[f] + rk[it];
        if constexpr (KEYS) sk[pos] = b0 + f;
        sv[pos] = SortEnt<E>::val(x[it], kb);
      }
    }
    __syncthreads();
    for (uint32_t q = t; q < cnt; q += S_THREADS) {
      if constexpr (KEYS) keys_out[start + q] = sk[q];
      vals_out[start + q] = sv[q];
    }
  } else if (cnt <= S2_BIG) {
    for (uint32_t e = t; e < cnt; e += S_THREADS) lds_rank_add(hist, SortEnt<E>::low(tmp[start + e]) & fmask);
    block_excl_scan(hist, nf, wsum);
    for (uint32_t f = t; f < nf; f += S_THREADS) offsets[b0 + f] = start + hist[f];
    __syncthreads();
    for (uint32_t e = t; e < cnt; e += S_THREADS) {
      const E x = tmp[start + e];
      const uint32_t f = SortEnt<E>::low(x) & fmask;
      const uint32_t pos = start + lds_rank_add(hist, f);
      if constexpr (KEYS) keys_out[pos] = b0 + f;
      vals_out[pos] = SortEnt<E>::val(x, kb);
    }
  } else {
    const uint32_t lo = p * S2_BIG, hi = min(lo + S2_BIG, cnt);
    for (uint32_t e = lo + t; e < hi; e += S_THREADS) lds_rank_add(hist, SortEnt<E>::low(tmp[start + e]) & fmask);
    __syncthreads();
    for (uint32_t f = t; f < nf; f += S_THREADS)
      if (hist[f]) atomicAdd(&fcount[b0 + f], hist[f]);
  }
}

constexpr uint32_t S2_SPLIT_GRID = 2048;
static __global__ void __launch_bounds__(1024) k_msm_s2_scan(const uint32_t* __restrict__ cbase,
                                                             const uint32_t* __restrict__ pbase, uint32_t NC,
                                                             uint32_t F, uint32_t T, uint32_t* __restrict__ fcount,
                                                             uint32_t* __restrict__ offsets) {
  extern __shared__ uint32_t hist[];
  __shared__ uint32_t wsum[17];
  if (pbase[NC] == NC) return;
  const uint32_t t = threadIdx.x;
  for (uint32_t H = blockIdx.x; H < NC; H += gridDim.x) {
    const uint32_t start = cbase[H], cnt = cbase[H + 1] - start;
    if (cnt <= S2_BIG) continue;
    const uint32_t b0 = H << F, nf = min(1u << F, T - b0);
    for (uint32_t f = t; f < nf; f += S_THREADS) hist[f] = fcount[b0 + f];
    block_excl_scan(hist, nf, wsum);
    for (uint32_t f = t; f < nf; f += S_THREADS) {
      offsets[b0 + f] = start + hist[f];
      fcount[b0 + f] = start + hist[f];
    }
    __syncthreads();
  }
}

template <class E, bool KEYS>
static __global__ void __launch_bounds__(1024) k_msm_s2_scatter(const E* __restrict__ tmp,
                                                                const uint32_t* __restrict__ cbase,
                                                                const uint32_t* __restrict__ pbase, uint32_t NC,
                                                                uint32_t F, uint32_t kb, uint32_t T,
                                                                uint32_t* __restrict__ fcursor,
                                                                uint32_t* __restrict__ keys_out,
                                                                uint32_t* __restrict__ vals_out) {
  extern __shared__ uint32_t s2_lds[];
  __shared__ uint32_t sh[2];
  const uint32_t t = threadIdx.x, parts = pbase[NC];
  if (parts == NC) return;
  for (uint32_t j = blockIdx.x; j < parts; j += gridDim.x) {
    s2_locate(pbase, NC, j, sh);
    const uint32_t H = sh[0], p = sh[1];
    const uint32_t start = cbase[H], cnt = cbase[H + 1] - start;
    __syncthreads();
    if (cnt <= S2_BIG) continue;
    const uint32_t b0 = H << F, nf = min(1u << F, T - b0), fmask = (1u << F) - 1;
    uint32_t* hist = s2_lds;
    uint32_t* cur = s2_lds + nf;
    for (uint32_t q = t; q < nf; q += S_THREADS) hist[q] = 0;
    __syncthreads();
    const uint32_t lo = p * S2_BIG, hi = min(lo + S2_BIG, cnt);
    for (uint32_t e = lo + t; e < hi; e += S_THREADS) lds_rank_add(hist, SortEnt<E>::low(tmp[start + e]) & fmask);
    __syncthreads();
    for (uint32_t f = t; f < nf; f += S_THREADS)
      if (hist[f]) cur[f] = atomicAdd(&fcursor[b0 + f], hist[f]);
    __syncthreads();
    for (uint32_t e = lo + t; e < hi; e += S_THREADS) {
      const E x = tmp[start + e];
      const uint32_t f = SortEnt<E>::low(x) & fmask;
      const uint32_t pos = lds_rank_add(cur, f);
      if constexpr (KEYS) keys_out[pos] = b0 + f;
      vals_out[pos] = SortEnt<E>::val(x, kb);
    }
    __syncthreads();
  }
}

template <class E, bool KEYS>
static int sort_passes(gm_ctx* ctx, Arena& arena, const SortGeom& g, size_t n, uint32_t W, uint32_t nb,
                       uint32_t shared_stride, const uint32_t* dig, const uint32_t* scount, uint32_t* keys_out,
                       uint32_t* vals_out, uint32_t* offsets) {
  hipStream_t st = ctx->stream;
  const uint32_t shift = g.F + g.G;
  int rc;
  DevBuf sbase, scursor, spbase, tmp;
  if ((rc = sbase.alloc(arena, 4 * ((size_t)g.NS + 1))) || (rc = scursor.alloc(arena, 4 * (size_t)g.NS)) ||
      (rc = spbase.alloc(arena, 4 * ((size_t)g.NS + 1))) || (rc = tmp.alloc(arena, sizeof(E) * g.M)))
    return rc;
  hipLaunchKernelGGL(k_msm_s1_scan, dim3(1), dim3(S_THREADS), 0, st, scount, g.NS, g.T, g.G ? SM_PART : S2_BIG,
                     sbase.as<uint32_t>(), scursor.as<uint32_t>(), spbase.as<uint32_t>(), offsets);
  const uint32_t nh = (!shared_stride && (1u << shift) <= nb) ? nb >> shift : g.NS;
  const size_t lds = 8 * (size_t)S1_PTS + sizeof(uint32_t) * (3 * (size_t)nh + 17);
  if (nh <= 4096 && lds <= device_lds_per_block(ctx->device)) {
    hipLaunchKernelGGL((k_msm_s1_scatter_st<E, S1_PPT>), dim3(blocks_for(n, S1_PTS), W), dim3(S_THREADS), lds, st, dig,
                       (uint32_t)n, nb, shared_stride, shift, g.NS, nh, scursor.as<uint32_t>(), tmp.as<E>());
    GM_HIP(hipGetLastError());
  } else {
    hipLaunchKernelGGL(k_msm_s1_scatter<E>, dim3(blocks_for(n, S1_PTS), W), dim3(S_THREADS),
                       2 * sizeof(uint32_t) * nh, st, dig, (uint32_t)n, nb, shared_stride, shift, g.NS, nh,
                       scursor.as<uint32_t>(), tmp.as<E>());
  }
  const E* fin = tmp.as<E>();
  const uint32_t *cbase = sbase.as<uint32_t>(), *pbase = spbase.as<uint32_t>();
  if (g.G) {
    DevBuf ccount, cb, ccur, cparts, pb, bsum, tmp2;
    if ((rc = ccount.alloc(arena, 4 * (size_t)g.NC)) || (rc = cb.alloc(arena, 4 * ((size_t)g.NC + 1))) ||
        (rc = ccur.alloc(arena, 4 * (size_t)g.NC)) || (rc = cparts.alloc(arena, 4 * (size_t)g.NC)) ||
        (rc = pb.alloc(arena, 4 * ((size_t)g.NC + 1))) || (rc = bsum.alloc(arena, 4 * scan_ws_words(g.NC))) ||
        (rc = tmp2.alloc(arena, sizeof(E) * g.M)))
      return rc;
    const size_t mparts = (size_t)g.NS + g.M / SM_PART + 1;
    GM_HIP(hipMemsetAsync(ccount.p, 0, 4 * (size_t)g.NC, st));
    hipLaunchKernelGGL(k_msm_sm_count<E>, dim3((unsigned)mparts), dim3(S_THREADS), 0, st, tmp.as<E>(),
                       sbase.as<uint32_t>(), spbase.as<uint32_t>(), g.NS, g.F, g.G, ccount.as<uint32_t>());
    hipLaunchKernelGGL(k_msm_sm_scan, dim3(g.NS), dim3(S_THREADS), 0, st, ccount.as<uint32_t>(), sbase.as<uint32_t>(),
                       g.G, g.NC, cb.as<uint32_t>(), ccur.as<uint32_t>(), cparts.as<uint32_t>());
    if ((rc = device_excl_scan(ctx, cparts.as<uint32_t>(), g.NC, pb.as<uint32_t>(), bsum.as<uint32_t>()))) return rc;
    hipLaunchKernelGGL(k_msm_sm_scatter<E>, dim3((unsigned)mparts), dim3(S_THREADS), 0, st, tmp.as<E>(),
                       sbase.as<uint32_t>(), spbase.as<uint32_t>(), g.NS, g.F, g.G, ccur.as<uint32_t>(),
                       tmp2.as<E>());
    fin = tmp2.as<E>();
    cbase = cb.as<uint32_t>();
    pbase = pb.as<uint32_t>();
  }
  DevBuf fcount;
  if ((rc = fcount.alloc(arena, 4 * (size_t)g.T))) return rc;
  const uint32_t nfmax = std::min<uint32_t>(1u << g.F, g.T);
  const size_t maxparts = (size_t)g.NC + g.M / S2_BIG + 1;
  GM_HIP(hipMemsetAsync(fcount.p, 0, sizeof(uint32_t) * g.T, st));
  hipLaunchKernelGGL((k_msm_s2_local<E, KEYS>), dim3((unsigned)maxparts), dim3(S_THREADS), s2_local_lds<KEYS>(nfmax),
                     st, fin, cbase, pbase, g.NC, g.F, shift, g.T, fcount.as<uint32_t>(), keys_out, vals_out, offsets);
  hipLaunchKernelGGL(k_msm_s2_scan, dim3(std::min<uint32_t>(g.NC, S2_SPLIT_GRID)), dim3(S_THREADS),
                     sizeof(uint32_t) * nfmax, st, cbase, pbase, g.NC, g.F, g.T, fcount.as<uint32_t>(), offsets);
  hipLaunchKernelGGL((k_msm_s2_scatter<E, KEYS>), dim3((unsigned)std::min<size_t>(maxparts, S2_SPLIT_GRID)),
                     dim3(S_THREADS), 2 * sizeof(uint32_t) * nfmax, st, fin, cbase, pbase, g.NC, g.F, shift, g.T,
                     fcount.as<uint32_t>(), keys_out, vals_out);
  GM_HIP(hipGetLastError());
  return GM_OK;
}

int msm_sort_digits(gm_ctx* ctx, Arena& arena, const SortGeom& g, size_t n, uint32_t W, uint32_t nb,
                    uint32_t shared_stride, const uint32_t* dig, const uint32_t* scount, uint32_t* keys_out,
                    uint32_t* vals_out, uint32_t* offsets) {
  if (g.NS == 0 || g.NS > 8192 || g.F > 13 || g.G > 10 || g.NC != (g.T + (1u << g.F) - 1) >> g.F ||
      g.NS != (g.T + (1u << (g.F + g.G)) - 1) >> (g.F + g.G)) {
    set_error("msm sort: bad geometry");
    return GM_ERR_INVALID;
  }
  const size_t vmax = shared_stride ? (size_t)W * shared_stride : n;
  if (g.compact && (vmax - 1) >> (31 - g.F - g.G)) {
    set_error("msm sort: values do not fit a compact entry");
    return GM_ERR_INVALID;
  }
  auto run = g.compact ? (keys_out ? sort_passes<uint32_t, true> : sort_passes<uint32_t, false>)
                       : (keys_out ? sort_passes<uint64_t, true> : sort_passes<uint64_t, false>);
  return run(ctx, arena, g, n, W, nb, shared_stride, dig, scount, keys_out, vals_out, offsets);
}

constexpr uint32_t PP_THREADS = 256, PP_PER = 2, PP_CLASSES = PIECE_MAX_LEN + 1, PP_COOP = 32, PP_BIG = 256;

__device__ __forceinline__ void pp_split(uint32_t len, uint32_t T, uint32_t& p, uint32_t& q, uint32_t& r) {
  p = (len + T - 1) / T;
  q = len / p;
  r = len - q * p;
}
__device__ __forceinline__ void pp_write(uint32_t b, uint32_t bs, uint32_t p, uint32_t q, uint32_t r, uint32_t i,
                                         uint32_t s0, uint32_t s1, uint32_t pb, uint4* __restrict__ pieces,
                                         uint32_t* __restrict__ partb) {
  const bool big = i < r;
  const uint32_t start = big ? bs + i * (q + 1) : bs + r * (q + 1) + (i - r) * q;
  pieces[big ? s1 + i : s0 + (i - r)] = make_uint4(start, big ? q + 1 : q, p == 1 ? b : PIECE_PART | (pb + i), 0u);
  if (p > 1) partb[pb + i] = b;
}

static __global__ void __launch_bounds__(PP_THREADS) k_msm_pp_hist(const uint32_t* __restrict__ offsets,
                                                                   uint32_t total, uint32_t T,
                                                                   uint32_t* __restrict__ hist) {
  __shared__ uint32_t h[PP_CLASSES];
  const uint32_t t = threadIdx.x;
  if (t < PP_CLASSES) h[t] = 0;
  __syncthreads();
  for (uint32_t k = 0; k < PP_PER; k++) {
    const uint32_t b = (blockIdx.x * PP_PER + k) * PP_THREADS + t;
    if (b >= total) break;
    const uint32_t len = offsets[b + 1] - offsets[b];
    if (!len) continue;
    uint32_t p, q, r;
    pp_split(len, T, p, q, r);
    atomicAdd(&h[q], p - r);
    if (r) atomicAdd(&h[q + 1], r);
  }
  __syncthreads();
  if (t < PP_CLASSES && h[t]) atomicAdd(&hist[t], h[t]);
}

static __global__ void __launch_bounds__(PP_THREADS) k_msm_pp_scan(const uint32_t* __restrict__ hist,
                                                                   uint32_t* __restrict__ cursor,
                                                                   uint32_t* __restrict__ pcount) {
  __shared__ uint32_t h[PP_CLASSES];
  const uint32_t t = threadIdx.x;
  if (t < PP_CLASSES) h[t] = hist[t];
  __syncthreads();
  if (t == 0) {
    uint32_t run = 0;
    for (int l = (int)PP_CLASSES - 1; l >= 0; l--) {
      const uint32_t c = h[l];
      h[l] = run;
      run += c;
    }
    pcount[0] = run;
    pcount[1] = 0;
  }
  __syncthreads();
  if (t < PP_CLASSES) cursor[t] = h[t];
}

static __global__ void __launch_bounds__(PP_THREADS) k_msm_pp_scatter(const uint32_t* __restrict__ offsets,
                                                                      uint32_t total, uint32_t T,
                                                                      uint32_t* __restrict__ cursor,
                                                                      uint32_t* __restrict__ pcount,
                                                                      uint4* __restrict__ pieces,
                                                                      uint32_t* __restrict__ pbase,
                                                                      uint32_t* __restrict__ partb) {
  __shared__ uint32_t cnt[PP_CLASSES], base[PP_CLASSES];
  __shared__ uint32_t nparts, part0, nbig;
  __shared__ uint32_t bigb[PP_BIG], bigs0[PP_BIG], bigs1[PP_BIG], bigpb[PP_BIG];
  const uint32_t t = threadIdx.x;
  if (t < PP_CLASSES) cnt[t] = 0;
  if (t == 0) {
    nparts = 0;
    nbig = 0;
  }
  __syncthreads();
  uint32_t loc[PP_PER];
#pragma unroll
  for (uint32_t k = 0; k < PP_PER; k++) {
    const uint32_t b = (blockIdx.x * PP_PER + k) * PP_THREADS + t;
    loc[k] = 0;
    if (b >= total) continue;
    const uint32_t len = offsets[b + 1] - offsets[b];
    if (!len) continue;
    uint32_t p, q, r;
    pp_split(len, T, p, q, r);
    atomicAdd(&cnt[q], p - r);
    if (r) atomicAdd(&cnt[q + 1], r);
    if (p > 1) loc[k] = atomicAdd(&nparts, p);
  }
  __syncthreads();
  if (t < PP_CLASSES) {
    if (cnt[t]) base[t] = atomicAdd(&cursor[t], cnt[t]);
    cnt[t] = 0;
  }
  if (t == 0 && nparts) part0 = atomicAdd(&pcount[1], nparts);
  __syncthreads();
#pragma unroll
  for (uint32_t k = 0; k < PP_PER; k++) {
    const uint32_t b = (blockIdx.x * PP_PER + k) * PP_THREADS + t;
    if (b >= total) continue;
    const uint32_t bs = offsets[b], len = offsets[b + 1] - bs;
    if (!len) continue;
    uint32_t p, q, r;
    pp_split(len, T, p, q, r);
    const uint32_t s0 = base[q] + atomicAdd(&cnt[q], p - r);
    const uint32_t s1 = r ? base[q + 1] + atomicAdd(&cnt[q + 1], r) : 0u;
    const uint32_t pb = p > 1 ? part0 + loc[k] : 0u;
    if (p > 1) pbase[b] = pb;
    if (p > PP_COOP) {
      const uint32_t e = atomicAdd(&nbig, 1u);
      if (e < PP_BIG) {
        bigb[e] = b;
        bigs0[e] = s0;
        bigs1[e] = s1;
        bigpb[e] = pb;
        continue;
      }
    }
    for (uint32_t i = 0; i < p; i++) pp_write(b, bs, p, q, r, i, s0, s1, pb, pieces, partb);
  }
  __syncthreads();
  const uint32_t nb = min(nbig, PP_BIG);
  for (uint32_t e = 0; e < nb; e++) {
    const uint32_t b = bigb[e], bs = offsets[b], len = offsets[b + 1] - bs;
    uint32_t p, q, r;
    pp_split(len, T, p, q, r);
    for (uint32_t i = t; i < p; i += PP_THREADS) pp_write(b, bs, p, q, r, i, bigs0[e], bigs1[e], bigpb[e], pieces, partb);
  }
}

int msm_piece_plan(gm_ctx* ctx, Arena& arena, MsmPlan& plan, uint32_t T) {
  if (T == 0 || T > PIECE_MAX_LEN) {
    set_error("msm piece plan: bad piece length");
    return GM_ERR_INVALID;
  }
  hipStream_t st = ctx->stream;
  const size_t M = plan.M, total = plan.total;
  plan.T = T;
  plan.max_pieces = M / T + std::min(total, M) + 1;
  plan.max_parts = std::min(2 * M / T, M / T + total) + 1;
  if (plan.max_pieces >= (size_t(1) << 31)) {
    set_error("msm piece plan: too many pieces");
    return GM_ERR_INVALID;
  }
  int rc;
  DevBuf pieces, pcount, pbase, partb, hist;
  if ((rc = pieces.alloc(arena, sizeof(uint4) * plan.max_pieces)) || (rc = pcount.alloc(arena, 16)) ||
      (rc = pbase.alloc(arena, sizeof(uint32_t) * total)) ||
      (rc = partb.alloc(arena, sizeof(uint32_t) * plan.max_parts)) ||
      (rc = hist.alloc(arena, sizeof(uint32_t) * 2 * PP_CLASSES)))
    return rc;
  uint32_t* h = hist.as<uint32_t>();
  const unsigned blocks = blocks_for(total, PP_THREADS * PP_PER);
  GM_HIP(hipMemsetAsync(h, 0, sizeof(uint32_t) * PP_CLASSES, st));
  hipLaunchKernelGGL(k_msm_pp_hist, dim3(blocks), dim3(PP_THREADS), 0, st, plan.offsets, plan.total, T, h);
  hipLaunchKernelGGL(k_msm_pp_scan, dim3(1), dim3(PP_THREADS), 0, st, h, h + PP_CLASSES, pcount.as<uint32_t>());
  hipLaunchKernelGGL(k_msm_pp_scatter, dim3(blocks), dim3(PP_THREADS), 0, st, plan.offsets, plan.total, T,
                     h + PP_CLASSES, pcount.as<uint32_t>(), pieces.as<uint4>(), pbase.as<uint32_t>(),
                     partb.as<uint32_t>());
  GM_HIP(hipGetLastError());
  plan.pieces = pieces.as<uint4>();
  plan.pcount = pcount.as<uint32_t>();
  plan.pbase = pbase.as<uint32_t>();
  plan.partb = partb.as<uint32_t>();
  return GM_OK;
}

MsmPrecomp msm_choose_precomp(size_t n, int bits) {
  MsmPrecomp best;
  double best_cost = 1e300;
  for (uint32_t c = 8; c <= 24; c++) {
    const uint32_t W = (uint32_t)((bits + 1 + c - 1) / c);
    const double cost = (double)n * W + 3.0 * (double)(1u << (c - 1));
    if (cost < best_cost) {
      best_cost = cost;
      best.c = c;
      best.W = W;
    }
  }
  best.stride = n;
  best.narrow = precomp_narrow(best.c, best.W, bits);
  return best;
}

}
```

Baseline: 748.8 Mpoints/s.

## Fuse piece-plan histogram into sort pass and merge control buffers and tail copies

Moves the piece-length class histogram out of a separate kernel and into the sort's second pass, accumulated in LDS and flushed to sharded global counters. The piece scatter kernel now does the class scan itself, which removes the hist and scan launches. The change also merges scount, the piece control words and the error/wsum tail into one allocation with a single memset. The last bitsum level writes gnark-format output directly, which drops the export kernel, and the two device-to-host copies become one. The aim is to cut launch and memset overhead at the cost of more complex sort kernels and extra per-block atomics.

```diff
diff --git a/gnark-icicle_amd/csrc/msm.hpp b/gnark-icicle_amd/csrc/msm.hpp
--- a/gnark-icicle_amd/csrc/msm.hpp
+++ b/gnark-icicle_amd/csrc/msm.hpp
@@ -24,9 +24,13 @@
   while (npts && ((npts - 1) >> (vb - 1))) vb++;
   return F + G + vb <= 32;
 }
+constexpr uint32_t PIECE_MAX_LEN = 128;
+constexpr uint32_t PP_CLASSES = PIECE_MAX_LEN + 1;
+constexpr uint32_t PP_SHARDS = 16;
+constexpr uint32_t PP_CTL_WORDS = (PP_SHARDS + 1) * PP_CLASSES + 4;
 int msm_sort_digits(gm_ctx* ctx, Arena& arena, const SortGeom& g, size_t n, uint32_t W, uint32_t nb,
                     uint32_t shared_stride, const uint32_t* dig, const uint32_t* scount, uint32_t* keys_out,
-                    uint32_t* vals_out, uint32_t* offsets);
+                    uint32_t* vals_out, uint32_t* offsets, uint32_t piece_len = 0, uint32_t* pphist = nullptr);
 
 constexpr uint32_t PRECOMP_LAYOUT = 2;
 struct MsmPrecomp {
@@ -166,9 +170,8 @@
   uint32_t* partb = nullptr;
 };
 constexpr uint32_t PIECE_PART = 0x80000000u;
-constexpr uint32_t PIECE_MAX_LEN = 128;
 uint32_t msm_piece_len(const gm_ctx* ctx, size_t M);
-int msm_piece_plan(gm_ctx* ctx, Arena& arena, MsmPlan& plan, uint32_t T);
+int msm_piece_plan(gm_ctx* ctx, Arena& arena, MsmPlan& plan, uint32_t T, uint32_t* ctl);
 template <class C>
 int msm_plan(gm_ctx* ctx, Arena& arena, const void* scalars_dev, size_t n, const MsmPrecomp* pre,
              MsmPlan& plan, bool glv = false, bool pieces = true, bool keys = true);
diff --git a/gnark-icicle_amd/csrc/msm_impl.hpp b/gnark-icicle_amd/csrc/msm_impl.hpp
--- a/gnark-icicle_amd/csrc/msm_impl.hpp
+++ b/gnark-icicle_amd/csrc/msm_impl.hpp
@@ -669,9 +669,17 @@
 }
 
 template <class F>
+GM_DEV void store_xyzz_gnark(uint32_t* __restrict__ o, const XYZZ<F>& r) {
+  Coord<F>::store_gnark(o, r.x);
+  Coord<F>::store_gnark(o + Coord<F>::WORDS, r.y);
+  Coord<F>::store_gnark(o + 2 * Coord<F>::WORDS, r.zz);
+  Coord<F>::store_gnark(o + 3 * Coord<F>::WORDS, r.zzz);
+}
+
+template <class F>
 __global__ void __launch_bounds__(BS_THREADS) k_msm_bitsum(const XYZZ<F>* __restrict__ in, uint32_t m,
                                                     uint32_t Qin, uint32_t NT, uint32_t lgNT,
-                                                    XYZZ<F>* __restrict__ out) {
+                                                    XYZZ<F>* __restrict__ out, uint32_t* __restrict__ gnark_out) {
   extern __shared__ __attribute__((aligned(16))) char smem_raw[];
   XYZZ<F>* X = reinterpret_cast<XYZZ<F>*>(smem_raw);
   const uint32_t groups = m / NT;
@@ -707,6 +715,11 @@
     __syncthreads();
   }
   const uint32_t Qout = Qin + lgNT;
+  if (gnark_out) {
+    for (uint32_t q = threadIdx.x; q < Qout; q += blockDim.x)
+      store_xyzz_gnark<F>(gnark_out + (((size_t)w * groups + j) * Qout + q) * 4 * Coord<F>::WORDS, X[q]);
+    return;
+  }
   XYZZ<F>* dst = out + ((size_t)w * groups + j) * Qout;
   for (uint32_t q = threadIdx.x; q < Qout; q += blockDim.x) dst[q] = X[q];
 }
@@ -716,17 +729,12 @@
                                                     uint32_t* __restrict__ out) {
   const uint32_t t = blockIdx.x * blockDim.x + threadIdx.x;
   if (t >= count) return;
-  uint32_t* o = out + (size_t)t * 4 * Coord<F>::WORDS;
-  const XYZZ<F> r = nodes[t];
-  Coord<F>::store_gnark(o, r.x);
-  Coord<F>::store_gnark(o + Coord<F>::WORDS, r.y);
-  Coord<F>::store_gnark(o + 2 * Coord<F>::WORDS, r.zz);
-  Coord<F>::store_gnark(o + 3 * Coord<F>::WORDS, r.zzz);
+  store_xyzz_gnark<F>(out + (size_t)t * 4 * Coord<F>::WORDS, nodes[t]);
 }
 
 template <class C>
-int msm_plan(gm_ctx* ctx, Arena& arena, const void* scalars_dev, size_t n, const MsmPrecomp* pre,
-             MsmPlan& plan, bool glv, bool pieces, bool keys) {
+int msm_plan_ctl(gm_ctx* ctx, Arena& arena, const void* scalars_dev, size_t n, const MsmPrecomp* pre,
+                 MsmPlan& plan, bool glv, bool pieces, bool keys, uint32_t tail_words, void** tail) {
   hipStream_t st = ctx->stream;
   plan = MsmPlan();
   plan.n = n;
@@ -758,12 +766,18 @@
   const size_t M = pg.M;
   const SortGeom& sg = pg.sg;
   int rc;
-  DevBuf dig, keys_out, vals_out, offsets, scount;
+  const uint32_t piece_len = pieces ? msm_piece_len(ctx, M) : 0u;
+  const size_t pph_at = sg.NS, errw_at = (pph_at + (pieces ? PP_CTL_WORDS : 0u) + 3) & ~size_t(3);
+  const size_t ctl_words = errw_at + (tail ? 4 : 0);
+  DevBuf dig, keys_out, vals_out, offsets, ctl;
   if ((rc = dig.alloc(arena, sizeof(uint32_t) * M)) || (keys && (rc = keys_out.alloc(arena, sizeof(uint32_t) * M))) ||
       (rc = vals_out.alloc(arena, sizeof(uint32_t) * M + 16)) ||
       (rc = offsets.alloc(arena, sizeof(uint32_t) * ((size_t)plan.total + 1))) ||
-      (rc = scount.alloc(arena, sizeof(uint32_t) * sg.NS)))
+      (rc = ctl.alloc(arena, sizeof(uint32_t) * (ctl_words + (tail ? (size_t)tail_words * pg.Wred * (2 + c) : 0)))))
     return rc;
+  uint32_t* const scount = ctl.as<uint32_t>();
+  uint32_t* const pphist = pieces ? scount + pph_at : nullptr;
+  if (tail) *tail = scount + errw_at;
   DigitGeom g;
   g.n = (uint32_t)n;
   g.c = c;
@@ -775,25 +789,25 @@
   g.F = sg.F + sg.G;
   {
     ProfScope ps(ctx, "msm_digits");
-    GM_HIP(hipMemsetAsync(scount.p, 0, sizeof(uint32_t) * sg.NS, st));
+    GM_HIP(hipMemsetAsync(ctl.p, 0, sizeof(uint32_t) * ctl_words, st));
     if constexpr (Glv<C>::ok) {
       if (glv)
         hipLaunchKernelGGL(k_msm_digits_glv<C>, dim3(blocks_for(n0, DG_THREADS * DG_PPT)), dim3(DG_THREADS),
                          sizeof(uint32_t) * sg.NS, st, reinterpret_cast<const uint32_t*>(scalars_dev), g,
-                           (uint32_t)n0, sg.NS, dig.as<uint32_t>(), scount.as<uint32_t>());
+                           (uint32_t)n0, sg.NS, dig.as<uint32_t>(), scount);
     }
     if (!glv)
       hipLaunchKernelGGL(k_msm_digits<typename C::Fr>, dim3(blocks_for(n, DG_THREADS * DG_PPT)), dim3(DG_THREADS),
                          sizeof(uint32_t) * sg.NS, st, reinterpret_cast<const uint32_t*>(scalars_dev), g, sg.NS,
-                         dig.as<uint32_t>(), scount.as<uint32_t>());
+                         dig.as<uint32_t>(), scount);
     GM_HIP(hipGetLastError());
   }
   {
     ProfScope ps(ctx, "msm_sort");
     if (ctx->profiling) ctx->stats[sg.compact ? "msm_sort_compact" : "msm_sort_wide"].count += 1;
-    if ((rc = msm_sort_digits(ctx, arena, sg, n, W, plan.nb, g.shared_stride, dig.as<uint32_t>(),
-                              scount.as<uint32_t>(), keys_out.as<uint32_t>(), vals_out.as<uint32_t>(),
-                              offsets.as<uint32_t>())))
+    if ((rc = msm_sort_digits(ctx, arena, sg, n, W, plan.nb, g.shared_stride, dig.as<uint32_t>(), scount,
+                              keys_out.as<uint32_t>(), vals_out.as<uint32_t>(), offsets.as<uint32_t>(), piece_len,
+                              pphist)))
       return rc;
   }
   plan.keys = keys_out.as<uint32_t>();
@@ -801,9 +815,15 @@
   plan.offsets = offsets.as<uint32_t>();
   if (pieces) {
     ProfScope ps(ctx, "msm_piece_plan");
-    if ((rc = msm_piece_plan(ctx, arena, plan, msm_piece_len(ctx, M)))) return rc;
+    if ((rc = msm_piece_plan(ctx, arena, plan, piece_len, pphist))) return rc;
   }
   return GM_OK;
+}
+
+template <class C>
+int msm_plan(gm_ctx* ctx, Arena& arena, const void* scalars_dev, size_t n, const MsmPrecomp* pre, MsmPlan& plan,
+             bool glv, bool pieces, bool keys) {
+  return msm_plan_ctl<C>(ctx, arena, scalars_dev, n, pre, plan, glv, pieces, keys, 0, nullptr);
 }
 
 template <class C, bool G2>
@@ -845,14 +865,15 @@
     if constexpr (kOneLane<DF>) {
       if (!pairs)
         hipLaunchKernelGGL(k_msm_bitsum<DF>, dim3(t.Wr * groups), dim3(BS_THREADS), sizeof(XYZZ<DF>) * NT * Q, st,
-                           cur, m, Q, NT, lg, nxt);
+                           cur, m, Q, NT, lg, nxt, lv + 1 == tg.levels ? (uint32_t*)t.wsum : nullptr);
     }
     Q += lg;
     m = groups;
     std::swap(cur, nxt);
   }
-  hipLaunchKernelGGL(k_msm_export<DF>, dim3(blocks_for((size_t)t.Wr * Q, 128)), dim3(128), 0, st, cur, t.Wr * Q,
-                     (uint32_t*)t.wsum);
+  if (pairs || tg.levels == 0)
+    hipLaunchKernelGGL(k_msm_export<DF>, dim3(blocks_for((size_t)t.Wr * Q, 128)), dim3(128), 0, st, cur, t.Wr * Q,
+                       (uint32_t*)t.wsum);
   GM_HIP(hipGetLastError());
   t.Q = Q;
   return GM_OK;
@@ -896,15 +917,15 @@
     if (int r = tail_pinned_acquire(ctx, 16 + wbytes, &t.stage, &t.stage_idx)) return r;
     t.stage_ctx = ctx;
   }
-  GM_HIP(hipMemcpyAsync(t.stage, t.errw, 16, hipMemcpyDeviceToHost, st));
-  GM_HIP(hipMemcpyAsync(t.stage + 16, t.wsum, wbytes, hipMemcpyDeviceToHost, st));
+  GM_HIP(hipMemcpyAsync(t.stage, t.errw, 16 + wbytes, hipMemcpyDeviceToHost, st));
   if (!t.done) GM_HIP(hipEventCreateWithFlags(&t.done, hipEventDisableTiming));
   GM_HIP(hipEventRecord(t.done, st));
   return GM_OK;
 }
 
 template <class C, bool G2>
-int msm_launch(gm_ctx* ctx, Arena& arena, const MsmPlan& plan, const void* points_internal, MsmTail& t) {
+int msm_launch_on(gm_ctx* ctx, Arena& arena, const MsmPlan& plan, const void* points_internal, MsmTail& t,
+                  void* tail) {
   using DF = typename GroupSel<C, G2>::DF;
   using HF = typename GroupSel<C, G2>::HF;
   hipStream_t st = ctx->stream;
@@ -939,22 +960,23 @@
   constexpr int WORDS = Coord<DF>::WORDS;
   static_assert(sizeof(HF) == 4 * WORDS, "host/device layout mismatch");
   const size_t nslices = G2 ? (t.M + t.K - 1) / t.K : plan.max_parts;
-  DevBuf buckets, nodes_a, nodes_b, wsum, errw, pfirst, plast;
-  if ((rc = errw.alloc(arena, 16)) || (rc = buckets.alloc(arena, sizeof(XYZZ<DF>) * (size_t)t.total)) ||
+  DevBuf buckets, nodes_a, nodes_b, errw, pfirst, plast;
+  errw.p = tail;
+  if ((!tail && (rc = errw.alloc(arena, 16 + sizeof(uint32_t) * 4 * WORDS * t.Wr * (2 + t.c)))) ||
+      (rc = buckets.alloc(arena, sizeof(XYZZ<DF>) * (size_t)t.total)) ||
       (rc = nodes_a.alloc(arena, sizeof(XYZZ<DF>) * 2 * (size_t)t.Wr * t.nseg)) ||
       (rc = nodes_b.alloc(arena, sizeof(XYZZ<DF>) * 2 * (size_t)t.Wr * t.nseg)) ||
-      (rc = wsum.alloc(arena, sizeof(uint32_t) * 4 * WORDS * t.Wr * (2 + t.c))) ||
       (rc = pfirst.alloc(arena, sizeof(XYZZ<DF>) * nslices)) ||
       (rc = plast.alloc(arena, G2 ? sizeof(XYZZ<DF>) * nslices : 16)))
     return rc;
   t.buckets = buckets.p;
   t.nodes_a = nodes_a.p;
   t.nodes_b = nodes_b.p;
-  t.wsum = wsum.p;
+  t.wsum = (uint8_t*)errw.p + 16;
   t.errw = errw.p;
   t.pfirst = pfirst.p;
   t.plast = plast.p;
-  GM_HIP(hipMemsetAsync(errw.p, 0, 16, st));
+  if (!tail) GM_HIP(hipMemsetAsync(errw.p, 0, 16, st));
   {
     if (ctx->acc_chain) {
       if (!ctx->acc_tail) GM_HIP(hipEventCreateWithFlags(&ctx->acc_tail, hipEventDisableTiming));
@@ -1029,6 +1051,11 @@
 }
 
 template <class C, bool G2>
+int msm_launch(gm_ctx* ctx, Arena& arena, const MsmPlan& plan, const void* points_internal, MsmTail& t) {
+  return msm_launch_on<C, G2>(ctx, arena, plan, points_internal, t, nullptr);
+}
+
+template <class C, bool G2>
 int msm_finish(gm_ctx* ctx, MsmTail& t, typename GroupSel<C, G2>::HF (&jac_out)[3]) {
   using HF = typename GroupSel<C, G2>::HF;
   using HJ = host::Jac<HF>;
@@ -1119,9 +1146,11 @@
     pts = ipts.p;
   }
   MsmPlan plan;
-  if ((rc = msm_plan<C>(ctx, arena, scalars_dev, n, pre, plan, glv, !G2, G2))) return rc;
+  void* tail = nullptr;
+  if ((rc = msm_plan_ctl<C>(ctx, arena, scalars_dev, n, pre, plan, glv, !G2, G2, 4 * Coord<DF>::WORDS, &tail)))
+    return rc;
   if (inputs_read) GM_HIP(hipEventRecord(inputs_read, ctx->stream));
-  return msm_launch<C, G2>(ctx, arena, plan, pts, t);
+  return msm_launch_on<C, G2>(ctx, arena, plan, pts, t, tail);
 }
 
 template <class C, bool G2>
diff --git a/gnark-icicle_amd/csrc/msm_sort.hip b/gnark-icicle_amd/csrc/msm_sort.hip
--- a/gnark-icicle_amd/csrc/msm_sort.hip
+++ b/gnark-icicle_amd/csrc/msm_sort.hip
@@ -42,10 +42,13 @@
                                                              uint32_t T, uint32_t psz, uint32_t* __restrict__ cbase,
                                                              uint32_t* __restrict__ ccursor,
                                                              uint32_t* __restrict__ pbase,
-                                                             uint32_t* __restrict__ offsets) {
+                                                             uint32_t* __restrict__ offsets, uint32_t F,
+                                                             uint32_t* __restrict__ fcount) {
   __shared__ uint32_t a[8192];
   __shared__ uint32_t wsum[17];
+  __shared__ uint32_t nsplit;
   const uint32_t t = threadIdx.x;
+  if (t == 0) nsplit = 0;
   for (uint32_t q = t; q < NC; q += S_THREADS) a[q] = ccount[q];
   const uint32_t total = block_excl_scan(a, NC, wsum);
   for (uint32_t q = t; q < NC; q += S_THREADS) {
@@ -61,6 +64,15 @@
   const uint32_t parts = block_excl_scan(a, NC, wsum);
   for (uint32_t q = t; q < NC; q += S_THREADS) pbase[q] = a[q];
   if (t == 0) pbase[NC] = parts;
+  if (!fcount || parts == NC) return;
+  __syncthreads();
+  for (uint32_t q = t; q < NC; q += S_THREADS)
+    if (ccount[q] > psz) a[atomicAdd(&nsplit, 1u)] = q;
+  __syncthreads();
+  for (uint32_t e = 0; e < nsplit; e++) {
+    const uint32_t b0 = a[e] << F, nf = min(1u << F, T - b0);
+    for (uint32_t f = t; f < nf; f += S_THREADS) fcount[b0 + f] = 0;
+  }
 }
 
 constexpr uint32_t S1_PPT = 8, S1_PTS = S_THREADS * S1_PPT;
@@ -188,10 +200,12 @@
                                                              const uint32_t* __restrict__ sbase, uint32_t G,
                                                              uint32_t NC, uint32_t* __restrict__ cbase,
                                                              uint32_t* __restrict__ ccursor,
-                                                             uint32_t* __restrict__ cparts) {
-  __shared__ uint32_t a[1024], wsum[17];
+                                                             uint32_t* __restrict__ cparts, uint32_t F, uint32_t T,
+                                                             uint32_t* __restrict__ fcount) {
+  __shared__ uint32_t a[1024], wsum[17], nsplit;
   const uint32_t s = blockIdx.x, t = threadIdx.x, H0 = s << G;
   const uint32_t nh = min(1u << G, NC - H0);
+  if (t == 0) nsplit = 0;
   for (uint32_t q = t; q < nh; q += S_THREADS) a[q] = ccount[H0 + q];
   block_excl_scan(a, nh, wsum);
   for (uint32_t q = t; q < nh; q += S_THREADS) {
@@ -201,6 +215,14 @@
     cparts[H0 + q] = c > S2_BIG ? (c + S2_BIG - 1) / S2_BIG : 1u;
   }
   if (t == 0 && H0 + nh == NC) cbase[NC] = sbase[s + 1];
+  __syncthreads();
+  for (uint32_t q = t; q < nh; q += S_THREADS)
+    if (ccount[H0 + q] > S2_BIG) a[atomicAdd(&nsplit, 1u)] = H0 + q;
+  __syncthreads();
+  for (uint32_t e = 0; e < nsplit; e++) {
+    const uint32_t b0 = a[e] << F, nf = min(1u << F, T - b0);
+    for (uint32_t f = t; f < nf; f += S_THREADS) fcount[b0 + f] = 0;
+  }
 }
 
 template <class E>
@@ -240,6 +262,28 @@
   }
 }
 
+__device__ __forceinline__ void pp_split(uint32_t len, uint32_t T, uint32_t& p, uint32_t& q, uint32_t& r) {
+  p = (len + T - 1) / T;
+  q = len / p;
+  r = len - q * p;
+}
+__device__ __forceinline__ void pp_count_lds(const uint32_t* cnt, uint32_t nf, uint32_t PT, uint32_t* pph) {
+  __syncthreads();
+  for (uint32_t f = threadIdx.x; f < nf; f += S_THREADS) {
+    const uint32_t len = cnt[f];
+    if (!len) continue;
+    uint32_t p, q, r;
+    pp_split(len, PT, p, q, r);
+    atomicAdd(&pph[q], p - r);
+    if (r) atomicAdd(&pph[q + 1], r);
+  }
+}
+__device__ __forceinline__ void pp_flush_lds(const uint32_t* pph, uint32_t* __restrict__ pphist) {
+  __syncthreads();
+  const uint32_t t = threadIdx.x;
+  if (t < PP_CLASSES && pph[t]) atomicAdd(&pphist[(blockIdx.x % PP_SHARDS) * PP_CLASSES + t], pph[t]);
+}
+
 template <bool KEYS>
 constexpr size_t s2_local_lds(uint32_t nf) {
   return sizeof(uint32_t) * (nf + (KEYS ? 2 : 1) * (size_t)S2_STAGE);
@@ -252,9 +296,10 @@
                                                               uint32_t* __restrict__ fcount,
                                                               uint32_t* __restrict__ keys_out,
                                                               uint32_t* __restrict__ vals_out,
-                                                              uint32_t* __restrict__ offsets) {
+                                                              uint32_t* __restrict__ offsets, uint32_t PT,
+                                                              uint32_t* __restrict__ pphist) {
   extern __shared__ uint32_t s2_lds[];
-  __shared__ uint32_t sh[2], wsum[17];
+  __shared__ uint32_t sh[2], wsum[17], pph[PP_CLASSES];
   const uint32_t j = blockIdx.x, t = threadIdx.x;
   const uint32_t parts = pbase[NC];
   const uint32_t cj0 = j < NC ? cbase[j] : 0u, cj1 = j < NC ? cbase[j + 1] : 0u;
@@ -275,6 +320,7 @@
   const uint32_t b0 = H << F, nf = min(1u << F, T - b0), fmask = (1u << F) - 1;
   uint32_t* hist = s2_lds;
   for (uint32_t q = t; q < nf; q += S_THREADS) hist[q] = 0;
+  if (PT && t < PP_CLASSES) pph[t] = 0;
   __syncthreads();
   if (cnt <= S2_STAGE) {
     constexpr uint32_t IPT = S2_STAGE / S_THREADS;
@@ -288,6 +334,7 @@
         rk[it] = lds_rank_add(hist, SortEnt<E>::low(x[it]) & fmask);
       }
     }
+    if (PT) pp_count_lds(hist, nf, PT, pph);
     block_excl_scan(hist, nf, wsum);
     for (uint32_t f = t; f < nf; f += S_THREADS) offsets[b0 + f] = start + hist[f];
     uint32_t* sv = s2_lds + nf;
@@ -309,6 +356,7 @@
     }
   } else if (cnt <= S2_BIG) {
     for (uint32_t e = t; e < cnt; e += S_THREADS) lds_rank_add(hist, SortEnt<E>::low(tmp[start + e]) & fmask);
+    if (PT) pp_count_lds(hist, nf, PT, pph);
     block_excl_scan(hist, nf, wsum);
     for (uint32_t f = t; f < nf; f += S_THREADS) offsets[b0 + f] = start + hist[f];
     __syncthreads();
@@ -325,23 +373,28 @@
     __syncthreads();
     for (uint32_t f = t; f < nf; f += S_THREADS)
       if (hist[f]) atomicAdd(&fcount[b0 + f], hist[f]);
-  }
+    return;
+  }
+  if (PT) pp_flush_lds(pph, pphist);
 }
 
 constexpr uint32_t S2_SPLIT_GRID = 2048;
 static __global__ void __launch_bounds__(1024) k_msm_s2_scan(const uint32_t* __restrict__ cbase,
                                                              const uint32_t* __restrict__ pbase, uint32_t NC,
                                                              uint32_t F, uint32_t T, uint32_t* __restrict__ fcount,
-                                                             uint32_t* __restrict__ offsets) {
+                                                             uint32_t* __restrict__ offsets, uint32_t PT,
+                                                             uint32_t* __restrict__ pphist) {
   extern __shared__ uint32_t hist[];
-  __shared__ uint32_t wsum[17];
+  __shared__ uint32_t wsum[17], pph[PP_CLASSES];
   if (pbase[NC] == NC) return;
   const uint32_t t = threadIdx.x;
+  if (PT && t < PP_CLASSES) pph[t] = 0;
   for (uint32_t H = blockIdx.x; H < NC; H += gridDim.x) {
     const uint32_t start = cbase[H], cnt = cbase[H + 1] - start;
     if (cnt <= S2_BIG) continue;
     const uint32_t b0 = H << F, nf = min(1u << F, T - b0);
     for (uint32_t f = t; f < nf; f += S_THREADS) hist[f] = fcount[b0 + f];
+    if (PT) pp_count_lds(hist, nf, PT, pph);
     block_excl_scan(hist, nf, wsum);
     for (uint32_t f = t; f < nf; f += S_THREADS) {
       offsets[b0 + f] = start + hist[f];
@@ -349,6 +402,7 @@
     }
     __syncthreads();
   }
+  if (PT) pp_flush_lds(pph, pphist);
 }
 
 template <class E, bool KEYS>
@@ -394,16 +448,18 @@
 template <class E, bool KEYS>
 static int sort_passes(gm_ctx* ctx, Arena& arena, const SortGeom& g, size_t n, uint32_t W, uint32_t nb,
                        uint32_t shared_stride, const uint32_t* dig, const uint32_t* scount, uint32_t* keys_out,
-                       uint32_t* vals_out, uint32_t* offsets) {
+                       uint32_t* vals_out, uint32_t* offsets, uint32_t piece_len, uint32_t* pphist) {
   hipStream_t st = ctx->stream;
   const uint32_t shift = g.F + g.G;
   int rc;
-  DevBuf sbase, scursor, spbase, tmp;
+  DevBuf sbase, scursor, spbase, tmp, fcount;
   if ((rc = sbase.alloc(arena, 4 * ((size_t)g.NS + 1))) || (rc = scursor.alloc(arena, 4 * (size_t)g.NS)) ||
-      (rc = spbase.alloc(arena, 4 * ((size_t)g.NS + 1))) || (rc = tmp.alloc(arena, sizeof(E) * g.M)))
+      (rc = spbase.alloc(arena, 4 * ((size_t)g.NS + 1))) || (rc = tmp.alloc(arena, sizeof(E) * g.M)) ||
+      (rc = fcount.alloc(arena, 4 * (size_t)g.T)))
     return rc;
   hipLaunchKernelGGL(k_msm_s1_scan, dim3(1), dim3(S_THREADS), 0, st, scount, g.NS, g.T, g.G ? SM_PART : S2_BIG,
-                     sbase.as<uint32_t>(), scursor.as<uint32_t>(), spbase.as<uint32_t>(), offsets);
+                     sbase.as<uint32_t>(), scursor.as<uint32_t>(), spbase.as<uint32_t>(), offsets, g.F,
+                     g.G ? nullptr : fcount.as<uint32_t>());
   const uint32_t nh = (!shared_stride && (1u << shift) <= nb) ? nb >> shift : g.NS;
   const size_t lds = 8 * (size_t)S1_PTS + sizeof(uint32_t) * (3 * (size_t)nh + 17);
   if (nh <= 4096 && lds <= device_lds_per_block(ctx->device)) {
@@ -429,7 +485,8 @@
     hipLaunchKernelGGL(k_msm_sm_count<E>, dim3((unsigned)mparts), dim3(S_THREADS), 0, st, tmp.as<E>(),
                        sbase.as<uint32_t>(), spbase.as<uint32_t>(), g.NS, g.F, g.G, ccount.as<uint32_t>());
     hipLaunchKernelGGL(k_msm_sm_scan, dim3(g.NS), dim3(S_THREADS), 0, st, ccount.as<uint32_t>(), sbase.as<uint32_t>(),
-                       g.G, g.NC, cb.as<uint32_t>(), ccur.as<uint32_t>(), cparts.as<uint32_t>());
+                       g.G, g.NC, cb.as<uint32_t>(), ccur.as<uint32_t>(), cparts.as<uint32_t>(), g.F, g.T,
+                       fcount.as<uint32_t>());
     if ((rc = device_excl_scan(ctx, cparts.as<uint32_t>(), g.NC, pb.as<uint32_t>(), bsum.as<uint32_t>()))) return rc;
     hipLaunchKernelGGL(k_msm_sm_scatter<E>, dim3((unsigned)mparts), dim3(S_THREADS), 0, st, tmp.as<E>(),
                        sbase.as<uint32_t>(), spbase.as<uint32_t>(), g.NS, g.F, g.G, ccur.as<uint32_t>(),
@@ -438,15 +495,14 @@
     cbase = cb.as<uint32_t>();
     pbase = pb.as<uint32_t>();
   }
-  DevBuf fcount;
-  if ((rc = fcount.alloc(arena, 4 * (size_t)g.T))) return rc;
   const uint32_t nfmax = std::min<uint32_t>(1u << g.F, g.T);
   const size_t maxparts = (size_t)g.NC + g.M / S2_BIG + 1;
-  GM_HIP(hipMemsetAsync(fcount.p, 0, sizeof(uint32_t) * g.T, st));
   hipLaunchKernelGGL((k_msm_s2_local<E, KEYS>), dim3((unsigned)maxparts), dim3(S_THREADS), s2_local_lds<KEYS>(nfmax),
-                     st, fin, cbase, pbase, g.NC, g.F, shift, g.T, fcount.as<uint32_t>(), keys_out, vals_out, offsets);
+                     st, fin, cbase, pbase, g.NC, g.F, shift, g.T, fcount.as<uint32_t>(), keys_out, vals_out, offsets,
+                     piece_len, pphist);
   hipLaunchKernelGGL(k_msm_s2_scan, dim3(std::min<uint32_t>(g.NC, S2_SPLIT_GRID)), dim3(S_THREADS),
-                     sizeof(uint32_t) * nfmax, st, cbase, pbase, g.NC, g.F, g.T, fcount.as<uint32_t>(), offsets);
+                     sizeof(uint32_t) * nfmax, st, cbase, pbase, g.NC, g.F, g.T, fcount.as<uint32_t>(), offsets,
+                     piece_len, pphist);
   hipLaunchKernelGGL((k_msm_s2_scatter<E, KEYS>), dim3((unsigned)std::min<size_t>(maxparts, S2_SPLIT_GRID)),
                      dim3(S_THREADS), 2 * sizeof(uint32_t) * nfmax, st, fin, cbase, pbase, g.NC, g.F, shift, g.T,
                      fcount.as<uint32_t>(), keys_out, vals_out);
@@ -456,7 +512,11 @@
 
 int msm_sort_digits(gm_ctx* ctx, Arena& arena, const SortGeom& g, size_t n, uint32_t W, uint32_t nb,
                     uint32_t shared_stride, const uint32_t* dig, const uint32_t* scount, uint32_t* keys_out,
-                    uint32_t* vals_out, uint32_t* offsets) {
+                    uint32_t* vals_out, uint32_t* offsets, uint32_t piece_len, uint32_t* pphist) {
+  if (piece_len > PIECE_MAX_LEN || (piece_len && !pphist)) {
+    set_error("msm sort: bad piece length");
+    return GM_ERR_INVALID;
+  }
   if (g.NS == 0 || g.NS > 8192 || g.F > 13 || g.G > 10 || g.NC != (g.T + (1u << g.F) - 1) >> g.F ||
       g.NS != (g.T + (1u << (g.F + g.G)) - 1) >> (g.F + g.G)) {
     set_error("msm sort: bad geometry");
@@ -469,16 +529,11 @@
   }
   auto run = g.compact ? (keys_out ? sort_passes<uint32_t, true> : sort_passes<uint32_t, false>)
                        : (keys_out ? sort_passes<uint64_t, true> : sort_passes<uint64_t, false>);
-  return run(ctx, arena, g, n, W, nb, shared_stride, dig, scount, keys_out, vals_out, offsets);
-}
-
-constexpr uint32_t PP_THREADS = 256, PP_PER = 2, PP_CLASSES = PIECE_MAX_LEN + 1, PP_COOP = 32, PP_BIG = 256;
-
-__device__ __forceinline__ void pp_split(uint32_t len, uint32_t T, uint32_t& p, uint32_t& q, uint32_t& r) {
-  p = (len + T - 1) / T;
-  q = len / p;
-  r = len - q * p;
-}
+  return run(ctx, arena, g, n, W, nb, shared_stride, dig, scount, keys_out, vals_out, offsets, piece_len, pphist);
+}
+
+constexpr uint32_t PP_THREADS = 256, PP_PER = 2, PP_COOP = 32, PP_BIG = 256;
+
 __device__ __forceinline__ void pp_write(uint32_t b, uint32_t bs, uint32_t p, uint32_t q, uint32_t r, uint32_t i,
                                          uint32_t s0, uint32_t s1, uint32_t pb, uint4* __restrict__ pieces,
                                          uint32_t* __restrict__ partb) {
@@ -488,57 +543,17 @@
   if (p > 1) partb[pb + i] = b;
 }
 
-static __global__ void __launch_bounds__(PP_THREADS) k_msm_pp_hist(const uint32_t* __restrict__ offsets,
-                                                                   uint32_t total, uint32_t T,
-                                                                   uint32_t* __restrict__ hist) {
-  __shared__ uint32_t h[PP_CLASSES];
-  const uint32_t t = threadIdx.x;
-  if (t < PP_CLASSES) h[t] = 0;
-  __syncthreads();
-  for (uint32_t k = 0; k < PP_PER; k++) {
-    const uint32_t b = (blockIdx.x * PP_PER + k) * PP_THREADS + t;
-    if (b >= total) break;
-    const uint32_t len = offsets[b + 1] - offsets[b];
-    if (!len) continue;
-    uint32_t p, q, r;
-    pp_split(len, T, p, q, r);
-    atomicAdd(&h[q], p - r);
-    if (r) atomicAdd(&h[q + 1], r);
-  }
-  __syncthreads();
-  if (t < PP_CLASSES && h[t]) atomicAdd(&hist[t], h[t]);
-}
-
-static __global__ void __launch_bounds__(PP_THREADS) k_msm_pp_scan(const uint32_t* __restrict__ hist,
-                                                                   uint32_t* __restrict__ cursor,
-                                                                   uint32_t* __restrict__ pcount) {
-  __shared__ uint32_t h[PP_CLASSES];
-  const uint32_t t = threadIdx.x;
-  if (t < PP_CLASSES) h[t] = hist[t];
-  __syncthreads();
-  if (t == 0) {
-    uint32_t run = 0;
-    for (int l = (int)PP_CLASSES - 1; l >= 0; l--) {
-      const uint32_t c = h[l];
-      h[l] = run;
-      run += c;
-    }
-    pcount[0] = run;
-    pcount[1] = 0;
-  }
-  __syncthreads();
-  if (t < PP_CLASSES) cursor[t] = h[t];
-}
-
 static __global__ void __launch_bounds__(PP_THREADS) k_msm_pp_scatter(const uint32_t* __restrict__ offsets,
                                                                       uint32_t total, uint32_t T,
+                                                                      const uint32_t* __restrict__ hist,
                                                                       uint32_t* __restrict__ cursor,
                                                                       uint32_t* __restrict__ pcount,
                                                                       uint4* __restrict__ pieces,
                                                                       uint32_t* __restrict__ pbase,
                                                                       uint32_t* __restrict__ partb) {
-  __shared__ uint32_t cnt[PP_CLASSES], base[PP_CLASSES];
-  __shared__ uint32_t nparts, part0, nbig;
+  __shared__ uint32_t cnt[PP_CLASSES], base[PP_CLASSES], cls[PP_CLASSES];
+  __shared__ uint32_t nparts, part0, nbig, wtot[2];
+  static_assert(PP_CLASSES > 128 && PP_CLASSES <= 192 && PP_THREADS >= 192, "class scan: three waves");
   __shared__ uint32_t bigb[PP_BIG], bigs0[PP_BIG], bigs1[PP_BIG], bigpb[PP_BIG];
   const uint32_t t = threadIdx.x;
   if (t < PP_CLASSES) cnt[t] = 0;
@@ -546,7 +561,17 @@
     nparts = 0;
     nbig = 0;
   }
-  __syncthreads();
+  uint32_t hv = 0;
+  if (t < PP_CLASSES)
+    for (uint32_t sh = 0; sh < PP_SHARDS; sh++) hv += hist[sh * PP_CLASSES + PP_CLASSES - 1 - t];
+  const uint32_t hinc = wave_incl_scan(hv);
+  if ((t & 63) == 63 && t < 128) wtot[t >> 6] = hinc;
+  __syncthreads();
+  if (t < PP_CLASSES) {
+    const uint32_t longer = hinc - hv + (t >= 64 ? wtot[0] : 0u) + (t >= 128 ? wtot[1] : 0u);
+    cls[PP_CLASSES - 1 - t] = longer;
+    if (t == PP_CLASSES - 1 && blockIdx.x == 0) pcount[0] = longer + hv;
+  }
   uint32_t loc[PP_PER];
 #pragma unroll
   for (uint32_t k = 0; k < PP_PER; k++) {
@@ -563,7 +588,7 @@
   }
   __syncthreads();
   if (t < PP_CLASSES) {
-    if (cnt[t]) base[t] = atomicAdd(&cursor[t], cnt[t]);
+    if (cnt[t]) base[t] = cls[t] + atomicAdd(&cursor[t], cnt[t]);
     cnt[t] = 0;
   }
   if (t == 0 && nparts) part0 = atomicAdd(&pcount[1], nparts);
@@ -602,7 +627,7 @@
   }
 }
 
-int msm_piece_plan(gm_ctx* ctx, Arena& arena, MsmPlan& plan, uint32_t T) {
+int msm_piece_plan(gm_ctx* ctx, Arena& arena, MsmPlan& plan, uint32_t T, uint32_t* ctl) {
   if (T == 0 || T > PIECE_MAX_LEN) {
     set_error("msm piece plan: bad piece length");
     return GM_ERR_INVALID;
@@ -617,23 +642,18 @@
     return GM_ERR_INVALID;
   }
   int rc;
-  DevBuf pieces, pcount, pbase, partb, hist;
-  if ((rc = pieces.alloc(arena, sizeof(uint4) * plan.max_pieces)) || (rc = pcount.alloc(arena, 16)) ||
+  DevBuf pieces, pbase, partb;
+  if ((rc = pieces.alloc(arena, sizeof(uint4) * plan.max_pieces)) ||
       (rc = pbase.alloc(arena, sizeof(uint32_t) * total)) ||
-      (rc = partb.alloc(arena, sizeof(uint32_t) * plan.max_parts)) ||
-      (rc = hist.alloc(arena, sizeof(uint32_t) * 2 * PP_CLASSES)))
+      (rc = partb.alloc(arena, sizeof(uint32_t) * plan.max_parts)))
     return rc;
-  uint32_t* h = hist.as<uint32_t>();
+  uint32_t *const cursor = ctl + PP_SHARDS * PP_CLASSES, *const pcount = cursor + PP_CLASSES;
   const unsigned blocks = blocks_for(total, PP_THREADS * PP_PER);
-  GM_HIP(hipMemsetAsync(h, 0, sizeof(uint32_t) * PP_CLASSES, st));
-  hipLaunchKernelGGL(k_msm_pp_hist, dim3(blocks), dim3(PP_THREADS), 0, st, plan.offsets, plan.total, T, h);
-  hipLaunchKernelGGL(k_msm_pp_scan, dim3(1), dim3(PP_THREADS), 0, st, h, h + PP_CLASSES, pcount.as<uint32_t>());
-  hipLaunchKernelGGL(k_msm_pp_scatter, dim3(blocks), dim3(PP_THREADS), 0, st, plan.offsets, plan.total, T,
-                     h + PP_CLASSES, pcount.as<uint32_t>(), pieces.as<uint4>(), pbase.as<uint32_t>(),
-                     partb.as<uint32_t>());
+  hipLaunchKernelGGL(k_msm_pp_scatter, dim3(blocks), dim3(PP_THREADS), 0, st, plan.offsets, plan.total, T, ctl, cursor,
+                     pcount, pieces.as<uint4>(), pbase.as<uint32_t>(), partb.as<uint32_t>());
   GM_HIP(hipGetLastError());
   plan.pieces = pieces.as<uint4>();
-  plan.pcount = pcount.as<uint32_t>();
+  plan.pcount = pcount;
   plan.pbase = pbase.as<uint32_t>();
   plan.partb = partb.as<uint32_t>();
   return GM_OK;
```

Measured after the change: 748.6 Mpoints/s, median of 2. Within noise of the previous version (-0.0%).
